# albanie/mcnCrossModalEmotions

Measured on AMD Instinct MI355X. Metric: distillation-step samples/sec (face+audio pair), higher is better.
Workload: dtype f32; 1 GPU; BASELINE config 4 shard: frozen resnet50 teacher fwd + VGGVox student fwd/bwd/SGD; per_gpu_batch=32, global_batch=32, face=224x224x3, teacher_batch=32, spectrogram=512x300x1, parallelism=dp1, weights=random-init (seeded), parameter_server=rccl-capi, streams=teacher one batch ahead on its own stream + wgrad side stream

## Files before the change

### include/xmodal.h

```cpp
#ifndef XMODAL_H
#define XMODAL_H
#include <stddef.h>
#ifdef __cplusplus
extern "C" {
#endif

enum {
  XM_OK = 0,
  XM_EINVAL = 1,
  XM_ENOMEM = 2,
  XM_EHIP = 3,
  XM_ETOOBIG = 4,
  XM_ENOTSUP = 5
};

enum { XM_POOL_MAX = 0, XM_POOL_AVG = 1 };
enum { XM_LOSS_SOFTMAXLOG = 0, XM_LOSS_CLASSERROR = 1 };
enum { XM_AGG_MAX = 0, XM_AGG_MEAN = 1, XM_AGG_PEAK = 2 };
enum { XM_MNR_CONVERGED = 0, XM_MNR_ITERLIMIT = 1, XM_MNR_NOTPD = 2, XM_MNR_BADINPUT = 3 };
enum { XM_ROC_OK = 0, XM_ROC_NAN = 1, XM_ROC_BADINPUT = 2 };

enum { XM_FUSE_RELU = 1, XM_BN_BATCH_MOMENTS = 2, XM_FUSE_SIGMOID = 4 };

int xm_version(void);
const char *xm_last_error(void);
int xm_device_alloc(void **ptr, size_t bytes);
int xm_device_free(void *ptr);
int xm_device_upload(void *dst_device, const void *src_host, size_t bytes);
int xm_device_download(void *dst_host, const void *src_device, size_t bytes);
int xm_device_synchronize(void);
enum { XM_EXEC_SINGLE_STREAM = 1 };
int xm_set_exec_hint(unsigned flags);
unsigned xm_get_exec_hint(void);
int xm_tune_load(const char *path);
int xm_tune_save(const char *path);
int xm_tune_entries(int *total, int *unsaved);
int xm_workspace_reserve(size_t bytes);
size_t xm_workspace_bytes(void);
int xm_workspace_reserve_stream(size_t bytes, void *stream);
unsigned long long xm_workspace_generation(void);
int xm_out_size(int in, int pad_a, int pad_b, int f, int dilate, int stride);

int xm_nnconv_forward(const float *x, int H, int W, int C, int N, const float *f, int FH, int FW,
                      int FC, int K, const float *b, float *y, int sy, int sx, int pt, int pb,
                      int pl, int pr, int dy, int dx, void *stream);
int xm_nnconv_forward_fused(const float *x, int H, int W, int C, int N, const float *f, int FH,
                            int FW, int FC, int K, const float *b, float *y, int sy, int sx,
                            int pt, int pb, int pl, int pr, int dy, int dx, const float *scale,
                            const float *shift, const float *residual, int flags, void *stream);
int xm_nnconv_forward_gated(const float *x, int H, int W, int C, int N, const float *f, int FH, int FW,
                            int FC, int K, const float *b, float *y, int sy, int sx, int pt, int pb,
                            int pl, int pr, int dy, int dx, const float *scale, const float *shift,
                            const float *gate, const float *residual, int flags, void *stream);
int xm_nnconv_forward_moments(const float *x, int H, int W, int C, int N, const float *f, int FH, int FW,
                              int FC, int K, const float *b, float *y, int sy, int sx, int pt, int pb,
                              int pl, int pr, int dy, int dx, float epsilon, float *moments_out, void *stream);
int xm_nnconv_backward(const float *x, int H, int W, int C, int N, const float *f, int FH, int FW,
                       int FC, int K, const float *dzdy, float *dx_out, float *df_out,
                       float *db_out, int sy, int sx, int pt, int pb, int pl, int pr, int dy,
                       int dx, void *stream);
int xm_nnconv_prepare_backward(int H, int W, int C, int N, const float *f, int FH, int FW, int FC, int K,
                               int sy, int sx, int pt, int pb, int pl, int pr, int dy, int dx, void *stream);
int xm_params_changed(void);
int xm_nnconv_backward_accum(const float *x, int H, int W, int C, int N, const float *f, int FH, int FW,
                             int FC, int K, const float *dzdy, float *dx_out, float *df_out,
                             float *db_out, int sy, int sx, int pt, int pb, int pl, int pr, int dy,
                             int dx, const float *dx_accum, void *stream);
int xm_nnconv_backward_filter_bnrelupool(const float *x, int H, int W, int C, int N, int FH, int FW, int FC, int K,
                                         int sy, int sx, int pt, int pb, int pl, int pr, int dy, int dx,
                                         const float *y, const float *bn_g, const float *bn_b, const float *moments,
                                         int train, int ph, int pw, int psy, int psx, int ppt, int ppb, int ppl,
                                         int ppr, const unsigned char *argmax, const float *y_pool,
                                         const float *dzdy_pool, float *dzdf_out, float *dzdb_out, float *dg_out,
                                         float *db_out, void *stream);
int xm_nnconv_bnorm_relu_pool_forward(const float *x, int H, int W, int C, int N, const float *f, int FH, int FW, int FC,
                                      int K, const float *bias, int sy, int sx, int pt, int pb, int pl, int pr, int dy, int dx,
                                      const float *bn_g, const float *bn_b, float epsilon, const float *moments_in, int ph,
                                      int pw, int psy, int psx, int ppt, int ppb, int ppl, int ppr, double *gram,
                                      float *y_pool, unsigned char *argmax, float *moments_out, void *stream);
int xm_stem_gram(const float *x, int H, int W, int N, int FH, int FW, int sy, int sx, int pt, int pb, int pl, int pr,
                 double *gram, void *stream);
int xm_stem_gram_moments(const double *gram, const float *f, const float *b, int FH, int FW, int K, float epsilon,
                         float *moments_out, void *stream);
int xm_nnconv_backward_filter_bnrelupool_gram(const float *x, int H, int W, int C, int N, const float *f, int FH, int FW,
                                              int FC, int K, const float *bias, int sy, int sx, int pt, int pb, int pl,
                                              int pr, int dy, int dx, const float *bn_g, const float *moments, int train,
                                              int ph, int pw, int psy, int psx, int ppt, int ppb, int ppl, int ppr,
                                              const unsigned char *argmax, const float *y_pool, const float *dzdy_pool,
                                              const double *gram, float *df_out, float *dbias_out, float *dg_out,
                                              float *db_out, void *stream);

int xm_nnpool_forward(const float *x, int H, int W, int C, int N, int ph, int pw, int sy, int sx,
                      int pt, int pb, int pl, int pr, int method, float *y, void *stream);
int xm_nnpool_backward(const float *x, int H, int W, int C, int N, int ph, int pw, int sy, int sx,
                       int pt, int pb, int pl, int pr, int method, const float *dzdy, float *dx_out,
                       void *stream);

int xm_nnpool_forward_argmax(const float *x, int H, int W, int C, int N, int ph, int pw, int sy,
                             int sx, int pt, int pb, int pl, int pr, float *y, unsigned char *argmax,
                             void *stream);
int xm_nnpool_backward_argmax(const unsigned char *argmax, int H, int W, int C, int N, int ph, int pw,
                              int sy, int sx, int pt, int pb, int pl, int pr, const float *dzdy,
                              float *dx_out, void *stream);
int xm_nnpool_global_avg_backward_accum(const float *dzdy, const float *accum, float *dx_out, int H, int W, int C, int N,
                                        void *stream);

int xm_nnbnorm_forward(const float *x, int H, int W, int C, int N, const float *g, const float *b,
                       float epsilon, const float *moments_in, float *y, float *moments_out,
                       void *stream);
int xm_nnbnorm_forward_fused(const float *x, int H, int W, int C, int N, const float *g,
                             const float *b, float epsilon, const float *moments_in, float *y,
                             float *moments_out, int flags, void *stream);
int xm_nnbnorm_backward(const float *x, int H, int W, int C, int N, const float *g, const float *b,
                        const float *dzdy, float epsilon, const float *moments_in, float *dx_out,
                        float *dg_out, float *db_out, float *moments_out, void *stream);
int xm_nnbnorm_backward_fused(const float *x, const float *y, int H, int W, int C, int N,
                              const float *g, const float *b, const float *dzdy, float epsilon,
                              const float *moments_in, float *dx_out, float *dg_out, float *db_out,
                              float *moments_out, int flags, void *stream);

int xm_nnbnorm_backward_dxsum(const float *x, const float *y, int H, int W, int C, int N,
                              const float *g, const float *b, const float *dzdy, float epsilon,
                              const float *moments_in, float *dx_out, float *dg_out, float *db_out,
                              float *moments_out, float *dxsum_out, int flags, void *stream);

int xm_nnbnorm_relu_pool_forward(const float *x, int H, int W, int C, int N, const float *g,
                                 const float *b, float epsilon, const float *moments_in, int ph, int pw,
                                 int sy, int sx, int pt, int pb, int pl, int pr, float *y_pool,
                                 unsigned char *argmax, float *moments_out, void *stream);
int xm_nnbnorm_relu_pool_backward(const float *x, int H, int W, int C, int N, const float *g,
                                  const float *b, const float *moments, int train, int ph, int pw,
                                  int sy, int sx, int pt, int pb, int pl, int pr,
                                  const unsigned char *argmax, const float *y_pool, const float *dzdy_pool,
                                  float *dx_out, float *dg_out, float *db_out, float *dxsum_out, void *stream);

int xm_nnrelu(const float *x, size_t n, float leak, const float *dzdy, float *y, void *stream);
int xm_nnsigmoid(const float *x, size_t n, const float *dzdy, float *y, void *stream);
int xm_sum2(const float *a, const float *b, size_t n, int flags, float *y, void *stream);
int xm_scale_axpy(const float *x, int HW, int CN, const float *a, const float *r, int flags,
                  float *y, void *stream);
int xm_scale_backward(const float *x, int HW, int CN, const float *a, const float *dzdy,
                      float *dx_out, float *da_out, void *stream);

int xm_nndropout_forward(const float *x, size_t n, float rate, unsigned long long seed, unsigned long long offset,
                         float *y, float *mask_out, void *stream);
// ... 107 lines not shown
```

### mcncrossmodalemotions_amd/_lib.py

```python
import ctypes as C
import os

import torch

_HERE = os.path.dirname(os.path.abspath(__file__))
SO_PATH = os.environ.get("XM_LIB_PATH") or os.path.join(_HERE, "libxmodal_hip.so")

c_fp = C.c_void_p
_i, _f, _sz, _vp = C.c_int, C.c_float, C.c_size_t, C.c_void_p

SIGNATURES = {
    "xm_version": [],
    "xm_last_error": [],
    "xm_tune_load": [C.c_char_p],
    "xm_tune_save": [C.c_char_p],
    "xm_tune_entries": [C.POINTER(C.c_int), C.POINTER(C.c_int)],
    "xm_set_exec_hint": [C.c_uint],
    "xm_get_exec_hint": [],
    "xm_workspace_reserve": [_sz],
    "xm_workspace_bytes": [],
    "xm_workspace_reserve_stream": [_sz, _vp],
    "xm_workspace_generation": [],
    "xm_device_alloc": [C.POINTER(C.c_void_p), _sz],
    "xm_device_free": [_vp],
    "xm_device_upload": [_vp, _vp, _sz],
    "xm_device_download": [_vp, _vp, _sz],
    "xm_device_synchronize": [],
    "xm_out_size": [_i] * 6,
    "xm_nnconv_forward": [c_fp] + [_i] * 4 + [c_fp] + [_i] * 4 + [c_fp, c_fp] + [_i] * 8 + [_vp],
    "xm_nnconv_forward_moments": [c_fp] + [_i] * 4 + [c_fp] + [_i] * 4 + [c_fp, c_fp] + [_i] * 8 + [_f, c_fp, _vp],
    "xm_nnconv_forward_gated": [c_fp] + [_i] * 4 + [c_fp] + [_i] * 4 + [c_fp, c_fp] + [_i] * 8 +
                               [c_fp, c_fp, c_fp, c_fp, _i, _vp],
    "xm_nnconv_forward_fused": [c_fp] + [_i] * 4 + [c_fp] + [_i] * 4 + [c_fp, c_fp] + [_i] * 8 +
                               [c_fp, c_fp, c_fp, _i, _vp],
    "xm_nnconv_backward": [c_fp] + [_i] * 4 + [c_fp] + [_i] * 4 + [c_fp, c_fp, c_fp, c_fp] +
                          [_i] * 8 + [_vp],
    "xm_nnconv_backward_accum": [c_fp] + [_i] * 4 + [c_fp] + [_i] * 4 + [c_fp, c_fp, c_fp, c_fp] +
                                [_i] * 8 + [c_fp, _vp],
    "xm_nnconv_prepare_backward": [_i] * 4 + [c_fp] + [_i] * 12 + [_vp],
    "xm_nnconv_backward_filter_bnrelupool": [c_fp] + [_i] * 16 + [c_fp, c_fp, c_fp, c_fp] + [_i] * 9 +
                                            [c_fp, c_fp, c_fp, c_fp, c_fp, c_fp, c_fp, _vp],
    "xm_stem_gram": [c_fp] + [_i] * 11 + [_vp, _vp],
    "xm_stem_gram_moments": [_vp, c_fp, c_fp, _i, _i, _i, _f, c_fp, _vp],
    "xm_nnconv_backward_filter_bnrelupool_gram": [c_fp] + [_i] * 4 + [c_fp] + [_i] * 4 + [c_fp] + [_i] * 8 +
                                                 [c_fp, c_fp] + [_i] * 9 + [c_fp, c_fp, c_fp, _vp, c_fp, c_fp, c_fp, c_fp, _vp],
    "xm_nnconv_bnorm_relu_pool_forward": [c_fp] + [_i] * 4 + [c_fp] + [_i] * 4 + [c_fp] + [_i] * 8 + [c_fp, c_fp, _f, c_fp] +
                                         [_i] * 8 + [_vp, c_fp, c_fp, c_fp, _vp],
    "xm_params_changed": [],
    "xm_nnpool_forward": [c_fp] + [_i] * 13 + [c_fp, _vp],
    "xm_nnpool_backward": [c_fp] + [_i] * 13 + [c_fp, c_fp, _vp],
    "xm_nnpool_forward_argmax": [c_fp] + [_i] * 12 + [c_fp, c_fp, _vp],
    "xm_nnpool_backward_argmax": [c_fp] + [_i] * 12 + [c_fp, c_fp, _vp],
    "xm_nnpool_global_avg_backward_accum": [c_fp, c_fp, c_fp, _i, _i, _i, _i, _vp],
    "xm_nnbnorm_forward": [c_fp] + [_i] * 4 + [c_fp, c_fp, _f, c_fp, c_fp, c_fp, _vp],
    "xm_nnbnorm_forward_fused": [c_fp] + [_i] * 4 + [c_fp, c_fp, _f, c_fp, c_fp, c_fp, _i, _vp],
    "xm_nnbnorm_backward": [c_fp] + [_i] * 4 + [c_fp, c_fp, c_fp, _f, c_fp, c_fp, c_fp, c_fp, c_fp,
                                               _vp],
    "xm_nnbnorm_backward_fused": [c_fp, c_fp] + [_i] * 4 + [c_fp, c_fp, c_fp, _f, c_fp, c_fp, c_fp,
                                                             c_fp, c_fp, _i, _vp],
    "xm_nnbnorm_backward_dxsum": [c_fp, c_fp] + [_i] * 4 + [c_fp, c_fp, c_fp, _f, c_fp, c_fp, c_fp,
                                                             c_fp, c_fp, c_fp, _i, _vp],
    "xm_nnbnorm_relu_pool_forward": [c_fp] + [_i] * 4 + [c_fp, c_fp, _f, c_fp] + [_i] * 8 +
                                    [c_fp, c_fp, c_fp, _vp],
    "xm_nnbnorm_relu_pool_backward": [c_fp] + [_i] * 4 + [c_fp, c_fp, c_fp, _i] + [_i] * 8 +
                                     [c_fp, c_fp, c_fp, c_fp, c_fp, c_fp, c_fp, _vp],
    "xm_nndropout_forward": [c_fp, _sz, _f, C.c_ulonglong, C.c_ulonglong, c_fp, c_fp, _vp],
    "xm_nndropout_apply": [c_fp, c_fp, _sz, c_fp, _vp],
    "xm_nnrelu": [c_fp, _sz, _f, c_fp, c_fp, _vp],
    "xm_nnsigmoid": [c_fp, _sz, c_fp, c_fp, _vp],
    "xm_sum2": [c_fp, c_fp, _sz, _i, c_fp, _vp],
    "xm_scale_axpy": [c_fp, _i, _i, c_fp, c_fp, _i, c_fp, _vp],
    "xm_scale_backward": [c_fp, _i, _i, c_fp, c_fp, c_fp, c_fp, _vp],
    "xm_se_squeeze_bn": [c_fp] + [_i] * 4 + [c_fp, c_fp, c_fp, c_fp, _vp],
    "xm_scale_axpy_bn": [c_fp] + [_i] * 4 + [c_fp, c_fp, c_fp, c_fp, c_fp, _i, c_fp, _vp],
    "xm_se_tail_backward_reduce": [c_fp, c_fp, c_fp] + [_i] * 4 + [c_fp, c_fp, c_fp, c_fp, c_fp, _vp],
    "xm_se_tail_backward_apply": [c_fp, c_fp, c_fp] + [_i] * 4 + [c_fp, c_fp, c_fp, c_fp, _i, c_fp, c_fp, c_fp, c_fp, c_fp, _vp],
    "xm_nnsoftmaxt": [c_fp, _i, _i, _i, _f, c_fp, _vp],
    "xm_nnsoftmaxt_backward": [c_fp, c_fp, _i, _i, _i, _f, c_fp, _vp],
    "xm_nnregloss": [c_fp, c_fp, _i, _i, _i, _f, c_fp, c_fp, c_fp, _vp],
    "xm_nnsoftmaxceloss": [c_fp, c_fp, _i, _i, _f, _i, c_fp, c_fp, c_fp, _vp],
    "xm_nnloss": [c_fp, c_fp, _i, _i, _i, c_fp, c_fp, _vp],
    "xm_sgd_update": [c_fp, c_fp, c_fp, _sz, _f, _f, _f, _f, _vp],
    "xm_average_update": [c_fp, c_fp, _sz, _f, _f, _vp],
    "xm_comm_unique_id": [_vp],
    "xm_comm_init": [_vp, _i, _i],
    "xm_allreduce_sum_f32": [c_fp, _sz, _vp],
    "xm_parserv_push": [c_fp, _sz, _vp],
    "xm_parserv_sync": [_vp],
    "xm_comm_count": [C.POINTER(C.c_int)],
    "xm_scale_f32": [c_fp, _sz, _f, _vp],
    "xm_comm_destroy": [],
    "xm_spec_rownorm": [c_fp, _i, _i, _i, c_fp, _vp],
    "xm_spec_magnitude": [c_fp, _i, _i, _i, c_fp, _vp],
    "xm_resample": [c_fp, _i, c_fp, _i, _i, _i, _i, c_fp, _i, _vp],
    "xm_wav_batch": [c_fp, C.c_longlong, c_fp, C.c_longlong, c_fp, c_fp, _i, c_fp, _i, _vp],
    "xm_spec_bucket_batch": [c_fp, C.c_longlong, c_fp, _i, _i, c_fp, _i, _i, _i, c_fp, _vp],
    "xm_aggregate_logits": [c_fp, _i, _i, c_fp, c_fp, _i, _i, c_fp, c_fp, _vp],
    "xm_max_label": [c_fp, _i, _i, c_fp, _vp],
    "xm_class_stats": [c_fp, c_fp, _i, _i, c_fp, c_fp, _vp],
    "xm_normalize_face": [c_fp, _i, _i, _i, C.POINTER(C.c_float), c_fp, _vp],
    "xm_crop_resize_face": [c_fp, _i, _i, _i, _f, _i, _i, C.POINTER(C.c_float), c_fp, _vp],
    "xm_nnaffinegrid": [c_fp, _i, _i, _i, c_fp, _vp],
    "xm_nnaffinegrid_backward": [c_fp, _i, _i, _i, c_fp, _vp],
    "xm_nnbilinearsampler": [c_fp] + [_i] * 4 + [c_fp] + [_i] * 3 + [c_fp, _vp],
    "xm_nnbilinearsampler_backward": [c_fp] + [_i] * 4 + [c_fp] + [_i] * 3 + [c_fp, c_fp, c_fp, _vp],
    "xm_ferplus_batch": [c_fp, _i, _i, _i, c_fp, c_fp, _i, _i, C.POINTER(C.c_float), c_fp, _vp],
    "xm_mnrfit": [c_fp, _i, _i, c_fp, _i, c_fp, c_fp, _i, _i, _i, C.c_double, c_fp, c_fp, c_fp, c_fp, _vp],
    "xm_mnrval": [c_fp, c_fp, _i, _i, _i, c_fp, c_fp, _i, _i, c_fp, c_fp, c_fp, c_fp, _vp],
    "xm_roc": [c_fp, _i, _i, c_fp, c_fp, c_fp, _i, _i, c_fp, c_fp, c_fp, c_fp, c_fp, c_fp, _vp],
    "xm_roc_launches": [],
    "xm_label_hist": [c_fp, _i, _i, _i, c_fp, _vp],
    "xm_group_rows": [c_fp, _i, c_fp, _i, _i, c_fp, c_fp, c_fp, _vp],
    "xm_gather_rows": [c_fp, _i, _i, _i, c_fp, _i, c_fp, _vp],
    "xm_scatter_rows": [c_fp, _i, _i, c_fp, _i, _i, c_fp, _vp],
    "xm_track_peaks": [c_fp, _i, _i, c_fp, c_fp, _i, c_fp, c_fp, c_fp, _vp],
    "xm_jpeg_plan": [_vp, _vp, _i, _vp, _vp, C.c_longlong, _vp, C.c_longlong, _vp],
    "xm_jpeg_decode_batch": [c_fp, C.c_longlong, c_fp, _i, c_fp, _i, c_fp, _i, _i, C.c_longlong, C.c_longlong, C.c_longlong,
                             c_fp, c_fp, _f, _i, _i, C.POINTER(C.c_float), c_fp, _vp],
    "xm_wav_plan": [_vp, _vp, _i, _vp, _i, C.c_longlong, _vp, _vp],
    "xm_wav_decode_batch": [c_fp, C.c_longlong, c_fp, _i, c_fp, C.c_longlong, _vp],
}
_RESTYPES = {"xm_get_exec_hint": C.c_uint, "xm_last_error": C.c_char_p, "xm_workspace_bytes": C.c_size_t,
             "xm_workspace_generation": C.c_ulonglong}
_DEBUG = {"xm_debug_set": [C.c_char_p, _i], "xm_debug_get": [C.c_char_p],
          "xm_prof_enable": [_i],
          "xm_prof_collect": [_i, C.POINTER(C.c_int), C.POINTER(C.c_double), C.POINTER(C.c_double),
                              C.POINTER(C.c_longlong)],
          "xm_prof_collect_bytes": [_i, C.POINTER(C.c_int), C.POINTER(C.c_double)],
          "xm_prof_kernel_name": [_i, C.c_char_p, _i]}
_SWITCHES = {"xm_debug_force_conv_cfg": "conv_cfg", "xm_debug_force_conv_splits": "conv_splits",
# ... 42 lines not shown
```

### mcncrossmodalemotions_amd/csrc/context.cpp

```cpp
#include <cstdlib>
#include <map>
#include <string>
#include <vector>

#include "xm_common.h"

namespace xm {
bool path_on(Path p) {
  static const char *const kEnv[kPathCount] = {"XM_NO_HYBRID",      "XM_NO_HALO",        "XM_NO_SKINNY",     "XM_NO_SKINNY4",
                                               "XM_NO_STEM",        "XM_NO_STEM_WGRAD",  "XM_NO_DMA",        "XM_NO_FUSED_STATS",
                                               "XM_DGRAD_MERGE",    "XM_NO_FAST_TRANSPOSE", "XM_NO_POOL_LDS", "XM_NO_POOL_PATCH",
                                               "XM_NO_POOL_POOLED", "XM_NO_W8", "XM_NO_WGRAD_PATCH", "XM_NO_WGRAD_PATCH_S2", "XM_NO_DGRAD_S2", "XM_NO_STEM3"};
  static bool on[kPathCount];
  static bool read = false;
  if (!read) {
    for (int i = 0; i < kPathCount; ++i) on[i] = getenv(kEnv[i]) == nullptr;
    read = true;
  }
  return on[p];
}

long long env_int(const char *name, long long dflt) {
  const char *e = getenv(name);
  return (e && *e) ? atoll(e) : dflt;
}
double env_double(const char *name, double dflt) {
  const char *e = getenv(name);
  return (e && *e) ? atof(e) : dflt;
}

static char g_err[512] = "";
char *err_buf() { return g_err; }

int fail(int code, const char *fmt, ...) {
  va_list ap;
  va_start(ap, fmt);
  vsnprintf(g_err, sizeof g_err, fmt, ap);
  va_end(ap);
  return code;
}

struct WsBuf {
  void *ptr = nullptr;
  size_t cap = 0;
};
static std::map<hipStream_t, WsBuf> g_ws;
static unsigned long long g_ws_generation = 0;

int ws_get(size_t bytes, void **ptr, hipStream_t stream) {
  WsBuf &w = g_ws[stream];
  if (bytes > w.cap) {
    size_t want = bytes + bytes / 4 + (1u << 20);
    static const bool verbose = getenv("XM_WS_VERBOSE") != nullptr;
    if (verbose) fprintf(stderr, "[xm ws] stream %p grow %zu -> %zu\n", (void *)stream, w.cap, want);
    ++g_ws_generation;
    if (w.ptr) {
      hipError_t e = hipDeviceSynchronize();
      if (e != hipSuccess) return fail(XM_EHIP, "hipDeviceSynchronize -> %s", hipGetErrorString(e));
      (void)hipFree(w.ptr);
      w.ptr = nullptr;
      w.cap = 0;
    }
    hipError_t e = hipMalloc(&w.ptr, want);
    if (e != hipSuccess) {
      w.ptr = nullptr;
      return fail(XM_ENOMEM, "workspace hipMalloc(%zu) -> %s", want, hipGetErrorString(e));
    }
    w.cap = want;
  }
  *ptr = w.ptr;
  return XM_OK;
}

static std::map<std::string, void *> g_tables;

const void *cached_device_table(const void *host, size_t bytes) {
  std::string key((const char *)host, bytes);
  auto it = g_tables.find(key);
  if (it != g_tables.end()) return it->second;
  void *d = nullptr;
  static const bool verbose = getenv("XM_WS_VERBOSE") != nullptr;
  if (verbose) fprintf(stderr, "[xm ws] new device table %zu bytes (#%zu)\n", bytes, g_tables.size());
  if (hipMalloc(&d, bytes) != hipSuccess) return nullptr;
  if (hipMemcpy(d, host, bytes, hipMemcpyHostToDevice) != hipSuccess) {
    (void)hipFree(d);
    return nullptr;
  }
  g_tables.emplace(std::move(key), d);
  return d;
}

}

extern "C" {

int xm_version(void) { return 114; }
const char *xm_last_error(void) { return xm::err_buf(); }

int xm_workspace_reserve(size_t bytes) {
  void *p;
  return xm::ws_get(bytes, &p, nullptr);
}
int xm_workspace_reserve_stream(size_t bytes, void *stream) {
  void *p;
  return xm::ws_get(bytes, &p, (hipStream_t)stream);
}
unsigned long long xm_workspace_generation(void) { return xm::g_ws_generation; }

int xm_device_alloc(void **ptr, size_t bytes) {
  if (!ptr) return xm::fail(XM_EINVAL, "device_alloc: NULL output");
  *ptr = nullptr;
  if (bytes == 0) return XM_OK;
  hipError_t e = hipMalloc(ptr, bytes);
  if (e != hipSuccess) return xm::fail(XM_ENOMEM, "hipMalloc(%zu) -> %s", bytes, hipGetErrorString(e));
  return XM_OK;
}
int xm_device_free(void *ptr) {
  if (!ptr) return XM_OK;
  hipError_t e = hipFree(ptr);
  if (e != hipSuccess) return xm::fail(XM_EHIP, "hipFree -> %s", hipGetErrorString(e));
  return XM_OK;
}
int xm_device_upload(void *dst_device, const void *src_host, size_t bytes) {
  if (bytes == 0) return XM_OK;
  if (!dst_device || !src_host) return xm::fail(XM_EINVAL, "device_upload: NULL pointer");
  hipError_t e = hipMemcpy(dst_device, src_host, bytes, hipMemcpyHostToDevice);
  if (e != hipSuccess) return xm::fail(XM_EHIP, "hipMemcpy(H2D, %zu) -> %s", bytes, hipGetErrorString(e));
  return XM_OK;
}
int xm_device_download(void *dst_host, const void *src_device, size_t bytes) {
  if (bytes == 0) return XM_OK;
  if (!dst_host || !src_device) return xm::fail(XM_EINVAL, "device_download: NULL pointer");
  hipError_t e = hipMemcpy(dst_host, src_device, bytes, hipMemcpyDeviceToHost);
  if (e != hipSuccess) return xm::fail(XM_EHIP, "hipMemcpy(D2H, %zu) -> %s", bytes, hipGetErrorString(e));
  return XM_OK;
}
int xm_device_synchronize(void) {
  hipError_t e = hipDeviceSynchronize();
  if (e != hipSuccess) return xm::fail(XM_EHIP, "hipDeviceSynchronize -> %s", hipGetErrorString(e));
  return XM_OK;
}
size_t xm_workspace_bytes(void) {
  size_t t = 0;
  for (auto &kv : xm::g_ws) t += kv.second.cap;
  return t;
}

int xm_out_size(int in, int pad_a, int pad_b, int f, int dilate, int stride) {
  return xm::out_size(in, pad_a, pad_b, f, dilate, stride);
}
}
```

### mcncrossmodalemotions_amd/csrc/conv.hip

```cpp
#include <dlfcn.h>

#include <algorithm>
#include <climits>
#include <cstdlib>
#include <map>
#include <string>
#include <vector>

#include "conv_kernels.h"
#include "stem_pool_kernels.h"

namespace xm {


__global__ void pad_filter_kernel(const float *__restrict__ f, float *__restrict__ o, int M, int R,
                                  int Rp) {
  size_t i = blockIdx.x * (size_t)blockDim.x + threadIdx.x;
  if (i >= (size_t)M * Rp) return;
  int r = (int)(i % Rp);
  size_t m = i / Rp;
  o[i] = r < R ? f[m * R + r] : 0.f;
}

struct PrepDiv {
  FastDiv tsT, T, tsNT, nT, nU, padc, rows;
};
__global__ void __launch_bounds__(256)
prep_dgrad_filter_kernel(const float *__restrict__ f, float *__restrict__ o, int FH, int FW, int FC,
                         int Kg, int u0, int ustep, int nU, int v0, int vstep, int nV, int lda,
                         int TS, int fold, PrepDiv dv) {
  extern __shared__ float tile[];
  const int T = FH * FW, nT = nU * nV;
  const int c0 = blockIdx.x * TS, k0 = blockIdx.y * TS;
  const int pitch = TS * T + 1;
  for (int i = threadIdx.x; i < TS * TS * T; i += 256) {
    int kl = (int)xm_div((uint32_t)i, dv.tsT), rem = i - kl * (TS * T);
    int cl = (int)xm_div((uint32_t)rem, dv.T);
    int c = c0 + cl, k = k0 + kl;
    tile[kl * pitch + rem] = (c < FC && k < Kg) ? f[(size_t)rem + (size_t)T * (c0 + (size_t)FC * k)] : 0.f;
  }
  __syncthreads();
  for (int i = threadIdx.x; i < TS * TS * nT; i += 256) {
    int cl = (int)xm_div((uint32_t)i, dv.tsNT), rem = i - cl * (TS * nT);
    int kl = (int)xm_div((uint32_t)rem, dv.nT), tt = rem - kl * nT;
    int iv = (int)xm_div((uint32_t)tt, dv.nU), iu = tt - iv * nU;
    int t = (u0 + iu * ustep) + FH * (v0 + iv * vstep);
    int c = c0 + cl, k = k0 + kl;
    if (c < FC && k < Kg) {
      size_t dst = fold ? (size_t)(iu + nU * c) * lda + (size_t)nV * k + iv
                        : (size_t)c * lda + (size_t)nT * k + tt;
      o[dst] = tile[kl * pitch + cl * T + t];
    }
  }
  if (blockIdx.y == 0) {
    const int used = (fold ? nV : nT) * Kg, rows = fold ? nU : 1;
    int padc = lda - used;
    for (int i = threadIdx.x; i < TS * rows * padc; i += 256) {
      int rl = (int)xm_div((uint32_t)i, dv.padc), rr = used + (i - rl * padc);
      int cl = (int)xm_div((uint32_t)rl, dv.rows), ul = rl - cl * rows;
      if (c0 + cl < FC) o[((size_t)(c0 + cl) * rows + ul) * lda + rr] = 0.f;
    }
  }
}

__global__ void __launch_bounds__(256)
transpose_filter_kernel(const float *__restrict__ f, float *__restrict__ o, int K, int R, int ldo) {
  __shared__ float tile[64][65];
  const int r0 = blockIdx.x * 64, k0 = blockIdx.y * 64;
  const int tx = threadIdx.x & 15, ty = threadIdx.x >> 4;
#pragma unroll
  for (int p = 0; p < 4; ++p) {
    const int k = k0 + ty + 16 * p, r = r0 + 4 * tx;
    float4 v = make_float4(0.f, 0.f, 0.f, 0.f);
    if (k < K && r < R) v = *reinterpret_cast<const float4 *>(f + (size_t)k * R + r);
    tile[ty + 16 * p][4 * tx + 0] = v.x;
    tile[ty + 16 * p][4 * tx + 1] = v.y;
    tile[ty + 16 * p][4 * tx + 2] = v.z;
    tile[ty + 16 * p][4 * tx + 3] = v.w;
  }
  __syncthreads();
#pragma unroll
  for (int p = 0; p < 4; ++p) {
    const int r = r0 + ty + 16 * p, k = k0 + 4 * tx;
    if (r < R && k < K) {
      float4 v = make_float4(tile[4 * tx + 0][ty + 16 * p], tile[4 * tx + 1][ty + 16 * p],
                             tile[4 * tx + 2][ty + 16 * p], tile[4 * tx + 3][ty + 16 * p]);
      *reinterpret_cast<float4 *>(o + (size_t)r * ldo + k) = v;
    }
  }
}

template <int ZL>
__global__ void __launch_bounds__(256)
reduce_splits_kernel(const float *__restrict__ part, float *__restrict__ out, size_t total, int splits,
                     size_t splitStride) {
  constexpr int OPB = 256 / ZL;
  const int ol = threadIdx.x % OPB, zl = threadIdx.x / OPB;
  const size_t i = blockIdx.x * (size_t)OPB + ol;
  float s0 = 0.f, s1 = 0.f, s2 = 0.f, s3 = 0.f;
  if (i < total) {
    const float *p = part + i;
    int z = zl;
    for (; z + 3 * ZL < splits; z += 4 * ZL) {
      s0 += p[(size_t)z * splitStride];
      s1 += p[(size_t)(z + ZL) * splitStride];
      s2 += p[(size_t)(z + 2 * ZL) * splitStride];
      s3 += p[(size_t)(z + 3 * ZL) * splitStride];
    }
    for (; z < splits; z += ZL) s0 += p[(size_t)z * splitStride];
  }
  float s = (s0 + s1) + (s2 + s3);
  if (ZL == 1) {
    if (i < total) out[i] = s;
    return;
  }
  __shared__ float red[256];
  red[threadIdx.x] = s;
  __syncthreads();
  if (zl == 0 && i < total) {
    float t = 0.f;
#pragma unroll
    for (int k = 0; k < ZL; ++k) t += red[k * OPB + ol];
    out[i] = t;
  }
}

static void launch_reduce_splits(const float *part, float *out, size_t total, int splits,
                                 size_t splitStride, hipStream_t st) {
  if (splits >= 64)
    hipLaunchKernelGGL(reduce_splits_kernel<16>, dim3((unsigned)((total + 15) / 16)), dim3(256), 0, st,
                       part, out, total, splits, splitStride);
  else if (splits >= 8)
    hipLaunchKernelGGL(reduce_splits_kernel<4>, dim3((unsigned)((total + 63) / 64)), dim3(256), 0, st,
                       part, out, total, splits, splitStride);
  else
    hipLaunchKernelGGL(reduce_splits_kernel<1>, dim3((unsigned)((total + 255) / 256)), dim3(256), 0, st,
                       part, out, total, splits, splitStride);
}

__global__ void __launch_bounds__(256)
bias_grad_partial_kernel(const float *__restrict__ dy, double *__restrict__ part, int HW, int K, int N,
                         int S, FastDiv divRun) {
  int k = blockIdx.x, sp = blockIdx.y;
  double s = 0.0;
  const bool vec = (HW & 3) == 0;
  const int nper = (N - sp + S - 1) / S;
  const int run = vec ? HW >> 2 : HW;
  for (int j = threadIdx.x; j < nper * run; j += 256) {
    const int nn = (int)xm_div((uint32_t)j, divRun), i = j - nn * run;
    const float *p = dy + (size_t)HW * (k + (size_t)K * (sp + nn * S));
    if (vec) {
      float4 v = reinterpret_cast<const float4 *>(p)[i];
      s += ((double)v.x + (double)v.y) + ((double)v.z + (double)v.w);
    } else {
      s += (double)p[i];
    }
  }
  __shared__ double red[4];
  s = xm_wave_sum_d(s);
  if ((threadIdx.x & 63) == 0) red[threadIdx.x >> 6] = s;
  __syncthreads();
  if (threadIdx.x == 0) part[(size_t)k * S + sp] = red[0] + red[1] + red[2] + red[3];
}

__global__ void __launch_bounds__(256)
bias_grad_finalize_kernel(const double *__restrict__ part, float *__restrict__ db, int K, int S) {
  const int k = blockIdx.x * 4 + (threadIdx.x >> 6), lane = threadIdx.x & 63;
  if (k >= K) return;
  double s = 0.0;
  for (int i = lane; i < S; i += 64) s += part[(size_t)k * S + i];
  s = xm_wave_sum_d(s);
  if (lane == 0) db[k] = (float)s;
// ... 957 lines not shown
  bool bigTaps, dma_ok;
};

static ConvGemmArgs forward_args(const Geo &g, int grp, const FwdOperands &o) {
  ConvGemmArgs a{};
  const size_t xoff = (size_t)grp * g.FC * g.H * g.W, yoff = (size_t)grp * g.Kg * g.Ho * g.Wo;
  a.A = o.A + (size_t)grp * g.Kg * o.lda, a.lda = o.lda, a.aBytes = (unsigned)((size_t)g.Kg * o.lda * 4);
  a.X = o.x + xoff, a.xBytes = (unsigned)((x_elements(g) - xoff) * 4), a.xSampleStride = g.H * g.W * g.C;
  a.Y = o.y + yoff, a.taps = o.taps, a.tapStride = (unsigned)((size_t)g.H * g.W * 4);
  a.bias = o.b ? o.b + grp * g.Kg : nullptr;
  a.scale = o.scale ? o.scale + grp * g.Kg : nullptr, a.shift = o.shift ? o.shift + grp * g.Kg : nullptr;
  a.resid = o.resid ? o.resid + yoff : nullptr, a.relu = o.relu;
  a.gate = o.gate ? o.gate + (size_t)grp * g.Kg : nullptr, a.gateStride = g.K;
  a.M = g.Kg, a.Rp = o.Rp, a.Rtrue = g.R;
  a.PI = g.Ho, a.PJ = g.Wo, a.NP = g.Ho * g.Wo * g.N;
  a.divPIJ = make_fastdiv((uint32_t)(g.Ho * g.Wo)), a.divPI = make_fastdiv((uint32_t)g.Ho);
  a.gsy = g.sy, a.gsx = g.sx, a.gh0 = -g.pt, a.gw0 = -g.pl, a.LimH = g.H, a.LimW = g.W;
  a.nU = o.bigTaps ? 1 : g.FH, a.nV = o.bigTaps ? 1 : g.FW;
  a.du0 = 0, a.dus = g.dy, a.dv0 = 0, a.dvs = g.dx;
  a.osy = 1, a.osx = 1, a.oh0 = 0, a.ow0 = 0, a.OH = g.Ho;
  a.oChanStride = g.Ho * g.Wo, a.oSampleStride = g.Ho * g.Wo * g.K, a.divMU = make_fastdiv(1), a.oUStride = 0;
  a.vecStore = ((g.Ho * g.Wo) % 4 == 0 && (((uintptr_t)a.Y | (uintptr_t)a.resid) & 15) == 0) ? 1 : 0;
  a.dmaOk = (o.dma_ok && a.vecStore) ? 1 : 0;
  return a;
}

struct FwdStats {
  bool ok;
  float *part;
  int ncg;
};
static ConvGemmArgs stats_args(const ConvGemmArgs &a, FwdStats &s, int ncg) {
  ConvGemmArgs aa = a;
  s.ncg = ncg;
  if (ncg > 0) aa.statPart = s.part, aa.statNcg = ncg;
  return aa;
}
static int forward_stats_reduce(const FwdStats &s, double *part2, float *moments_out, int K, int NP, float eps, hipStream_t st) {
  const int S = std::max(1, std::min(64, s.ncg / 768));
  hipLaunchKernelGGL(conv_stats_reduce_kernel, dim3((K + 7) / 8, S), dim3(256), 0, st, s.part, moments_out, part2, K, s.ncg, S,
                     (double)NP, eps);
  XM_LAUNCH_CHECK();
  if (S > 1) {
    hipLaunchKernelGGL(conv_stats_finalize2_kernel, dim3((K + 255) / 256), dim3(256), 0, st, part2, moments_out, K, S,
                       (double)NP, eps);
    XM_LAUNCH_CHECK();
  }
  return XM_OK;
}

static int forward_run(const Geo &g, const ConvGemmArgs &a, const float *x, const float *f, int mode, float *slab,
                       FwdStats &s, hipStream_t st) {
  auto gemm = [&](int ci) {
    int sp;
    ci = a.dmaOk ? ci : base_cfg(ci);
    gemm_slab_floats(a, ci, &sp);
    const bool carry = s.ok && sp == 1 && g_force_splits <= 1;
    ConvGemmArgs aa = stats_args(a, s, carry ? (a.NP + kCfgs[ci].bn() - 1) / kCfgs[ci].bn() : 0);
    const int rc_ = launch_gemm(aa, mode, ci, sp, slab, st);
    if (aa.statPart) s.ncg = aa.statNcg;
    return rc_;
  };
  const TuneKey key = tune_key_forward(0, g, a.M, a.NP, a.Rp, mode + (s.ok ? 4 : 0));
  const int ci = tune_cfg(key, pick_cfg(a.M, a.NP, a.Rp / kBK), st, gemm, a.dmaOk ? kNumCfg : kNumBaseCfg, w8_skip(a.M, a.NP));
  if (stem_ok(a, g, x, s.ok)) {
    auto arm = [&](int h) { return h ? launch_stem(stats_args(a, s, s.ok ? stem_grid(a.NP) : 0), f, g.R, st) : gemm(ci); };
    return arm(select_arm(7, key, st, 2, kOneChallenger, kHaloMargin, g_force_stem, arm));
  }
  if (stem3_ok(a, g, x, s.ok)) {
    auto arm = [&](int h) { return h ? launch_stem3(a, f, g.R, st) : gemm(ci); };
    return arm(select_arm(12, key, st, 2, kOneChallenger, kHaloMargin, g_force_stem3, arm));
  }
  ConvGemmArgs ah = a;
  const int hneed = forced_tiling() ? 0 : halo_setup(ah, g.N);
  const bool hok[4] = {true, halo_var_ok(ah, hneed, 0), halo_var_ok(ah, hneed, 1), halo_var_ok(ah, hneed, 2)};
  auto arm = [&](int h) {
    if (!h) return gemm(ci);
    const bool carry = s.ok && halo_splits(ah, h - 1) == 1;
    return launch_halo(stats_args(ah, s, carry ? (a.NP + 127) / 128 : 0), h - 1, slab, st);
  };
  return arm(select_arm(4, key, st, 4, hok, kHaloMargin, halo_forced(hok), arm));
}

static int conv_forward(const float *x, const float *f, const float *b, float *y, const Geo &g,
                        const float *scale, const float *shift, const float *resid, int relu,
                        hipStream_t st, float *moments_out = nullptr, float eps = 0.f, const float *gate = nullptr) {
  const bool padded = (g.pt | g.pb | g.pl | g.pr) != 0;
  const bool bigTaps = g.FH * g.FW > 63;
  if (bigTaps && padded)
    return fail(XM_ENOTSUP, "vl_nnconv: padded filters with more than 63 spatial taps (%dx%d) are not built",
                g.FH, g.FW);
  const int Rp = (g.R + kBK - 1) / kBK * kBK;
  const bool need_pad = (g.R % kBK) != 0 || ((uintptr_t)f & 15);
  const int mode = (padded || Rp != g.R) ? 1 : 0;
  const int NP = g.Ho * g.Wo * g.N;
  const size_t slabf = slab_floats(g.Kg, NP, Rp, kNumCfg, g.FH, g.FW, g.R);
  const bool dma_ok = !need_pad && mode == 0 && g.FH == 1 && g.FW == 1 && g.sy == 1 && g.sx == 1 && g.dy == 1 &&
                      g.dx == 1 && (g.H * g.W) % 4 == 0 && ((uintptr_t)x & 15) == 0 && ((uintptr_t)f & 15) == 0 &&
                      g.R % kBK == 0 && path_on(kPathDma);
  const bool want_stats = moments_out != nullptr && g.G == 1 && path_on(kPathFusedStats);
  const size_t statf = want_stats ? (size_t)2 * g.K * std::max((NP + 31) / 32, stem_grid(NP)) : 0;
  const size_t stat2 = want_stats ? (size_t)2 * g.K * 64 : 0;
  WsCarver ws;
  int rc = ws.init(WsCarver::need(need_pad ? (size_t)g.K * Rp : 0, 4) + WsCarver::need(slabf, 4) +
                       WsCarver::need(statf, 4) + WsCarver::need(stat2, 8), st);
  if (rc) return rc;
  FwdOperands o{x, f, b, scale, shift, resid, gate, y, device_taps(fwd_tap_table(g, Rp, bigTaps)), g.R, Rp, relu, bigTaps, dma_ok};
  if (!o.taps) return fail(XM_ENOMEM, "vl_nnconv: tap table allocation failed");
  if (need_pad) {
    float *Ap = ws.take<float>((size_t)g.K * Rp);
    size_t n = (size_t)g.K * Rp;
    hipLaunchKernelGGL(pad_filter_kernel, dim3((unsigned)((n + 255) / 256)), dim3(256), 0, st, f, Ap,
                       g.K, g.R, Rp);
    XM_LAUNCH_CHECK();
    o.A = Ap;
    o.lda = Rp;
  }
  float *slab = slabf ? ws.take<float>(slabf) : nullptr;
  float *statp = statf ? ws.take<float>(statf) : nullptr;
  double *statp2 = stat2 ? ws.take<double>(stat2) : nullptr;
  bool stats_done = false;
  for (int grp = 0; grp < g.G; ++grp) {
    ConvGemmArgs a = forward_args(g, grp, o);
    FwdStats s{want_stats && a.vecStore && !relu && !resid, statp, 0};
    if (s.ok) a.dmaOk = 0;
    rc = forward_run(g, a, x, f, mode, slab, s, st);
    if (rc) return rc;
    if (s.ncg > 0) {
      rc = forward_stats_reduce(s, statp2, moments_out, g.K, NP, eps, st);
      if (rc) return rc;
      stats_done = true;
    }
  }
  if (moments_out && !stats_done) return bn_batch_moments(y, g.Ho, g.Wo, g.K, g.N, eps, moments_out, st);
  return XM_OK;
}

struct PrepKey {
  const float *f;
  int FH, FW, FC, K, sy, sx, dy, dx, pt, pl, H, W, fold;
  bool operator<(const PrepKey &o) const { return memcmp(this, &o, sizeof(PrepKey)) < 0; }
};
struct PrepEntry {
  float *buf = nullptr;
  size_t bytes = 0;
  unsigned long long version = ~0ull;
  hipEvent_t ev = nullptr;
  hipStream_t st = nullptr;
};
static std::map<PrepKey, PrepEntry> g_prep;
unsigned long long g_param_version = 1;
static PrepKey prep_key(const float *f, const Geo &g, bool fold) {
  PrepKey k;
  memset(&k, 0, sizeof k);
  k.f = f, k.FH = g.FH, k.FW = g.FW, k.FC = g.FC, k.K = g.K, k.sy = g.sy, k.sx = g.sx, k.dy = g.dy, k.dx = g.dx;
  k.pt = g.pt, k.pl = g.pl, k.H = g.H, k.W = g.W, k.fold = fold ? 1 : 0;
  return k;
}

static int g_force_dgrad_s2 = -1;
static bool dgrad_s2_ok(const Geo &g, const float *dzdy, const float *dxo, const float *accum) {
  if (!path_on(kPathDgradS2) || g_force_dgrad_s2 == 0 || forced_tiling()) return false;
  if (!dgrad_s2_can(g, (uintptr_t)dzdy, (uintptr_t)dxo, accum != nullptr)) return false;
  if (g_force_dgrad_s2 == 1) return true;
  static const long long min_blocks = env_int("XM_DGRAD_S2_MIN_BLOCKS", 6 * 768);
  const long long per_sample = (long long)((g.W + 3) / 4 + (g.W + 2) / 4) * (((g.H + 1) / 2 + 63) / 64) * ((g.C + kDgS2Rows - 1) / kDgS2Rows);
  return per_sample * g.N >= min_blocks;
}
static int launch_dgrad_s2(const float *dzdy, const float *f, float *dxo, const Geo &g, hipStream_t st) {
  DgradS2Args a{};
  a.dY = dzdy;
  a.dX = dxo;
  a.dyBytes = (unsigned)((size_t)g.Ho * g.Wo * g.K * g.N * 4);
  a.C = g.C, a.K = g.K, a.H = g.H, a.W = g.W, a.Ho = g.Ho, a.Wo = g.Wo;
  a.pl = g.pl;
  a.nbm = (g.C + kDgS2Rows - 1) / kDgS2Rows;
  a.nkg = g.K / 8;
  a.nmt = ((g.H + 1) / 2 + 63) / 64;
  int blocks = 0;
  for (int px = 0; px < 2; ++px) {
    a.xfirst[px] = ((px - g.pl) % 2 + 2) % 2;
    const int ncols = a.xfirst[px] < g.W ? (g.W - a.xfirst[px] + 1) / 2 : 0;
    a.ncg[px] = (ncols + 1) / 2;
    a.nv[px] = px == 0 ? 3 : 2;
    blocks += a.ncg[px] * a.nmt * a.nbm;
  }
  const size_t fdFloats = (size_t)a.nbm * 2 * 3 * a.nkg * kDgS2Tile;
  WsCarver ws;
  int rc = ws.init(WsCarver::need(fdFloats, 4), st);
  if (rc) return rc;
  float *Fd = ws.take<float>(fdFloats);
  a.Fd = Fd;
  hipLaunchKernelGGL(prep_dgrad_s2_kernel, dim3((unsigned)std::min<size_t>((fdFloats + 255) / 256, 2048)), dim3(256), 0, st, f,
                     Fd, g.C, g.K, a.nbm, a.nkg, g.pl);
  XM_LAUNCH_CHECK();
  {
    ProfScope ps(11 * 100, 2.0 * g.K * (double)g.Ho * g.Wo * g.N * g.R, st,
                 (double)a.dyBytes + 4.0 * g.K * g.R + 4.0 * g.C * (double)g.H * g.W * g.N);
    hipLaunchKernelGGL(conv_dgrad_s2_kernel<1>, dim3((unsigned)(blocks * g.N)), dim3(256), 0, st, a);
  }
  XM_LAUNCH_CHECK();
  return XM_OK;
}

struct DgradFilters {
  char *base = nullptr;
  std::vector<size_t> off;
  float *slab = nullptr;
  float *of(const Geo &g, const DgradClass &c, size_t ic, int grp, bool foldH) const {
    return (float *)(base + off[ic]) + (size_t)grp * g.FC * (foldH ? g.FH : 1) * c.Rp;
  }
};
static bool dgrad_pure_transpose(const Geo &g, const DgradClass &c, bool foldH, const float *f, const float *Ag) {
  const int Rrows = g.FC * (foldH ? g.FH : 1);
  return g.FW == 1 && ((foldH && c.nU == g.FH && c.nV == 1) || (g.FH == 1 && !foldH)) && c.Rp == g.Kg &&
         (Rrows & 3) == 0 && (g.Kg & 3) == 0 && g.G == 1 && (((uintptr_t)f | (uintptr_t)Ag) & 15) == 0 &&
         path_on(kPathFastTranspose);
}
static int launch_dgrad_filter(const float *f, float *Ag, const Geo &g, const DgradClass &c, int grp, bool foldH, hipStream_t st) {
  if (dgrad_pure_transpose(g, c, foldH, f, Ag)) {
    const int Rrows = g.FC * (foldH ? g.FH : 1);
    hipLaunchKernelGGL(transpose_filter_kernel, dim3((Rrows + 63) / 64, (g.Kg + 63) / 64), dim3(256), 0, st, f, Ag,
                       g.Kg, Rrows, c.Rp);
    XM_LAUNCH_CHECK();
    return XM_OK;
  }
  const int T = g.FH * g.FW;
  const int TS = T <= 14 ? 32 : (T <= 56 ? 16 : 8);
  size_t lds = sizeof(float) * (size_t)TS * (TS * T + 1);
  const int nT = c.nU * c.nV, used = (foldH ? c.nV : nT) * g.Kg;
  PrepDiv pd;
  pd.tsT = make_fastdiv((uint32_t)(TS * T)), pd.T = make_fastdiv((uint32_t)T);
  pd.tsNT = make_fastdiv((uint32_t)std::max(1, TS * nT)), pd.nT = make_fastdiv((uint32_t)std::max(1, nT));
  pd.nU = make_fastdiv((uint32_t)std::max(1, c.nU));
  pd.padc = make_fastdiv((uint32_t)std::max(1, c.Rp - used));
  pd.rows = make_fastdiv((uint32_t)(foldH ? std::max(1, c.nU) : 1));
  hipLaunchKernelGGL(prep_dgrad_filter_kernel, dim3((g.FC + TS - 1) / TS, (g.Kg + TS - 1) / TS),
                     dim3(256), lds, st, f + (size_t)g.R * g.Kg * grp, Ag, g.FH, g.FW, g.FC, g.Kg,
                     c.u0, c.ustep, c.nU, c.v0, c.vstep, c.nV, c.Rp, TS, foldH ? 1 : 0, pd);
  XM_LAUNCH_CHECK();
  return XM_OK;
}

static int dgrad_filter_operand(const float *f, const Geo &g, const std::vector<DgradClass> &cls, bool foldH,
                                size_t slab_floats, bool prepare_only, hipStream_t st, WsCarver &ws, DgradFilters &F) {
  size_t abytes = 0;
  for (const DgradClass &c : cls) {
    F.off.push_back(abytes);
    abytes += WsCarver::need((size_t)g.FC * (foldH ? g.FH : 1) * c.Rp * g.G, 4);
  }
  const PrepKey pkey = prep_key(f, g, foldH);
  PrepEntry *pe = nullptr;
  bool have_prepared = false;
  if (prepare_only) {
    pe = &g_prep[pkey];
    if (pe->bytes < abytes) {
      if (pe->buf) {
        XM_HIP(hipDeviceSynchronize());
        (void)hipFree(pe->buf);
      }
      pe->buf = nullptr;
      XM_HIP(hipMalloc((void **)&pe->buf, abytes));
      pe->bytes = abytes;
    }
    if (!pe->ev) XM_HIP(hipEventCreateWithFlags(&pe->ev, hipEventDisableTiming));
  } else {
    auto it = g_prep.find(pkey);
    if (it != g_prep.end() && it->second.version == g_param_version && it->second.bytes >= abytes) {
      pe = &it->second;
      have_prepared = true;
      if (pe->st != st) XM_HIP(hipStreamWaitEvent(st, pe->ev, 0));
    }
  }
  int rc = ws.init((pe ? 0 : abytes) + WsCarver::need(slab_floats, 4), st);
  if (rc) return rc;
  F.base = pe ? (char *)pe->buf : ws.base;
  F.slab = slab_floats ? (float *)(ws.base + (pe ? 0 : abytes)) : nullptr;
  for (size_t ic = 0; ic < cls.size() && !have_prepared; ++ic)
    for (int grp = 0; grp < g.G; ++grp) {
      rc = launch_dgrad_filter(f, F.of(g, cls[ic], ic, grp, foldH), g, cls[ic], grp, foldH, st);
      if (rc) return rc;
    }
  if (prepare_only) {
    pe->version = g_param_version;
    pe->st = st;
    XM_HIP(hipEventRecord(pe->ev, st));
  }
  return XM_OK;
}

struct DgradOperands {
  const float *dzdy, *accum;
  float *dxo;
  bool foldH;
  double pair_total;
};

static ConvGemmArgs dgrad_args(const Geo &g, const DgradClass &c, int grp, const DgradOperands &o, const float *Ag,
                               const int2 *taps) {
  const bool foldH = o.foldH;
  const DgradGather q = dgrad_gather(g, c, foldH);
  ConvGemmArgs a{};
  const size_t xoff = (size_t)grp * g.Kg * g.Ho * g.Wo, yoff = (size_t)grp * g.FC * g.H * g.W;
  a.A = Ag, a.lda = c.Rp, a.taps = taps;
  a.X = o.dzdy + xoff, a.xBytes = (unsigned)((y_elements(g) - xoff) * 4), a.xSampleStride = g.Ho * g.Wo * g.K;
  a.Y = o.dxo + yoff, a.resid = o.accum ? o.accum + yoff : nullptr;
  a.M = foldH ? g.FC * g.FH : g.FC, a.Rp = c.Rp, a.Rtrue = c.Rc;
  a.PI = foldH ? 1 : c.PI, a.PJ = c.PJ, a.NP = a.PI * c.PJ * g.N;
  a.divPIJ = make_fastdiv((uint32_t)(a.PI * c.PJ)), a.divPI = make_fastdiv((uint32_t)a.PI);
  a.gsy = 1, a.gsx = 1, a.gh0 = q.gh0, a.gw0 = q.gw0, a.LimH = g.Ho, a.LimW = g.Wo;
  a.nU = q.nU, a.nV = c.nV, a.du0 = q.du0, a.dus = q.dus, a.dv0 = q.dv0, a.dvs = q.dvs;
  a.osy = foldH ? 0 : g.sy, a.oh0 = foldH ? 0 : c.hi0;
  a.osx = g.sx, a.ow0 = c.wi0, a.OH = g.H;
  a.oChanStride = g.H * g.W, a.oSampleStride = g.H * g.W * g.C;
  a.divMU = make_fastdiv(foldH ? (uint32_t)g.FH : 1u), a.oUStride = foldH ? 1 : 0;
  a.vecStore = (!foldH && g.sy == 1 && g.sx == 1 && (c.PI * c.PJ) % 4 == 0 && c.PI == g.H &&
                c.PJ == g.W && (((uintptr_t)a.Y | (uintptr_t)a.resid) & 15) == 0) ? 1 : 0;
  a.algoFlops = 2.0 * g.Ho * g.Wo * (double)g.N * g.Kg * g.R * ((double)a.NP * c.Rc) / o.pair_total;
  return a;
}

static bool dgrad_as_skinny_fc(const Geo &g, bool pure_t, bool foldH, const float *accum, Geo &gs) {
  if (!pure_t || foldH || accum || g.FH != 1 || g.sy != 1 || g.sx != 1 || (g.pt | g.pb | g.pl | g.pr) != 0 ||
      g.H * g.W != 1 || (g.FC & 3) != 0 || g.N > 512 || forced_tiling())
    return false;
  gs = g;
  gs.C = gs.FC = g.Kg;
  gs.K = gs.Kg = g.FC;
  gs.R = g.Kg;
  return fc_skinny_ok(gs, true);
}

static int dgrad_run_class(const Geo &g, const DgradClass &c, const ConvGemmArgs &a, bool foldH, float *slab, hipStream_t st) {
  auto gemm = [&](int ci) {
    int sp;
    gemm_slab_floats(a, ci, &sp);
    ConvGemmArgs aa = a;
    return launch_gemm(aa, 1, ci, sp, slab, st);
  };
  const TuneKey key = tune_key_class_dgrad(1, g, c, a.M, a.NP, a.PI);
  const int ci = tune_cfg(key, pick_cfg(a.M, a.NP, c.Rp / kBK), st, gemm, kNumBaseCfg, w8_skip(a.M, a.NP));
  ConvGemmArgs ah = a;
  const int hneed = (!forced_tiling() && !foldH) ? halo_setup_padded(ah, g.N) : 0;
  const bool hok[4] = {true, halo_var_ok(ah, hneed, 0), halo_var_ok(ah, hneed, 1), halo_var_ok(ah, hneed, 2)};
  auto arm = [&](int h) { return h ? launch_halo(ah, h - 1, slab, st) : gemm(ci); };
  return arm(select_arm(5, key, st, 4, hok, kHaloMargin, halo_forced(hok), arm));
}

static bool dgrad_merge_ok(const Geo &g, const std::vector<DgradClass> &cls, bool foldH) {
  if (g.G != 1 || foldH || cls.size() < 2 || cls.size() > 4 || g_force_splits != 0 || !path_on(kPathDgradMerge)) return false;
  long long tiles = 0;
  for (const DgradClass &c : cls) tiles += (long long)((g.FC + 127) / 128) * (((long long)c.PI * c.PJ * g.N + 255) / 256);
  return tiles >= 512;
}

static int dgrad_run_merged(const Geo &g, const std::vector<ConvGemmArgs> &merged, hipStream_t st) {
  auto gemm = [&](int ci) { return launch_gemm_multi(merged, ci, st); };
  long long npSum = 0;
  int rpMax = 0;
  for (const ConvGemmArgs &a : merged) {
    npSum += a.NP;
    rpMax = std::max(rpMax, a.Rp);
  }
  const TuneKey key = tune_key_merged_dgrad(3, g, merged[0].M, npSum, rpMax, (int)merged.size());
  const int ci = tune_cfg(key, pick_cfg(merged[0].M, npSum, rpMax / kBK), st, gemm, kNumBaseCfg, w8_skip(merged[0].M, npSum));
  std::vector<ConvGemmArgs> mh = merged;
  bool hok[4] = {true, g_force_cfg < 0, g_force_cfg < 0, g_force_cfg < 0};
  for (ConvGemmArgs &a : mh) {
    const int need = hok[1] || hok[2] || hok[3] ? halo_setup_padded(a, g.N) : 0;
    for (int v = 0; v < 3; ++v) hok[v + 1] = hok[v + 1] && halo_var_ok(a, need, v);
  }
  if (!hok[3]) {
    bool all = g_force_cfg < 0;
    for (ConvGemmArgs &a : mh) {
      ConvGemmArgs t = a;
      const int need = all ? halo_setup_padded(t, g.N) : 0;
      all = all && need > 0 && need <= 1024 && t.M % 96 == 0;
    }
    hok[3] = all && !hok[2];
  }
  auto arm = [&](int h) { return h ? launch_halo_multi(mh, h - 1, st) : gemm(ci); };
  return arm(select_arm(6, key, st, 4, hok, kHaloMargin, halo_forced(hok), arm));
}

static int conv_dgrad(const float *f, const float *dzdy, float *dxo, const Geo &g, hipStream_t st,
                      const float *accum = nullptr, bool prepare_only = false) {
  if (dgrad_s2_ok(g, dzdy, dxo, accum)) {
    if (prepare_only) return XM_OK;
    return launch_dgrad_s2(dzdy, f, dxo, g, st);
  }
  const bool foldH = dgrad_fold_h(g);
  bool covers_all = true;
  const std::vector<DgradClass> cls = dgrad_classes(g, foldH, &covers_all);
  if (!prepare_only && (!covers_all || cls.empty())) {
    const size_t bytes = sizeof(float) * x_elements(g);
    if (accum)
      XM_HIP(hipMemcpyAsync(dxo, accum, bytes, hipMemcpyDeviceToDevice, st));
    else
      XM_HIP(hipMemsetAsync(dxo, 0, bytes, st));
  }
  if (cls.empty()) return XM_OK;
  for (const DgradClass &c : cls)
    if (c.nU * c.nV > 63)
      return fail(XM_ENOTSUP, "vl_nnconv: more than 63 spatial taps per stride class is not built");
  size_t slab_max = 0;
  for (const DgradClass &c : cls)
    slab_max = std::max(slab_max, slab_floats(foldH ? g.FC * g.FH : g.FC, (foldH ? 1 : c.PI) * c.PJ * g.N, c.Rp, kNumBaseCfg,
                                              foldH ? 0 : c.nU, foldH ? 0 : c.nV, c.Rc));
  WsCarver ws;
  DgradFilters F;
  int rc = dgrad_filter_operand(f, g, cls, foldH, slab_max, prepare_only, st, ws, F);
  if (rc) return rc;
  std::vector<const int2 *> taps;
  for (const DgradClass &c : cls) {
    taps.push_back(device_taps(dgrad_tap_table(g, c, foldH)));
    if (!taps.back()) return fail(XM_ENOMEM, "vl_nnconv: tap table allocation failed");
  }
  if (prepare_only) return XM_OK;
  DgradOperands o{dzdy, accum, dxo, foldH, 0.0};
  for (const DgradClass &c : cls) o.pair_total += (double)(foldH ? 1 : c.PI) * c.PJ * g.N * c.Rc;
  const bool merge = dgrad_merge_ok(g, cls, foldH);
  std::vector<ConvGemmArgs> merged;
  for (size_t ic = 0; ic < cls.size(); ++ic)
    for (int grp = 0; grp < g.G; ++grp) {
      const DgradClass &c = cls[ic];
      const float *Ag = F.of(g, c, ic, grp, foldH);
      Geo gs;
      if (dgrad_as_skinny_fc(g, dgrad_pure_transpose(g, c, foldH, f, Ag), foldH, accum, gs)) {
        rc = fc_skinny_forward(dzdy, Ag, nullptr, dxo, gs, 0, st);
        if (rc) return rc;
        continue;
      }
      const ConvGemmArgs a = dgrad_args(g, c, grp, o, Ag, taps[ic]);
      if (merge) {
        merged.push_back(a);
        continue;
      }
      rc = dgrad_run_class(g, c, a, foldH, F.slab, st);
      if (rc) return rc;
    }
  return merge ? dgrad_run_merged(g, merged, st) : XM_OK;
}

static int wgrad_run(const float *x, const float *dzdy, float *dfo, const Geo &g, int ci, float *part,
                     hipStream_t st) {
  ci = wgrad_cfg(ci);
  const Cfg &c = kCfgs[ci];
  const int NP = g.Ho * g.Wo * g.N;
  const int nkt = (NP + kBK - 1) / kBK;
  const int nbm = (g.Kg + c.bm() - 1) / c.bm(), nbn = (g.R + c.bn() - 1) / c.bn();
  const int Rn = nbn * c.bn();
  const int tiles = nbm * nbn;
  const int slots = 256 * (c.bm() * c.bn() >= 128 * 128 ? 2 : (c.bm() * c.bn() >= 64 * 128 ? 3 : 6));
  int splits = std::max(1, std::min(nkt / 8, slots / tiles));
  splits = std::min(splits, 1024);
  int tps = (nkt + splits - 1) / splits;
  splits = (nkt + tps - 1) / tps;
  const int4 *taps = device_taps(wgrad_tap_table(g, Rn));
  if (!taps) return fail(XM_ENOMEM, "vl_nnconv: tap table allocation failed");
  const size_t slab = (size_t)g.Kg * g.R;
  for (int grp = 0; grp < g.G; ++grp) {
    WgradArgs a{};
    const size_t xoff = (size_t)grp * g.FC * g.H * g.W, doff = (size_t)grp * g.Kg * g.Ho * g.Wo;
    float *dst = dfo + (size_t)grp * g.Kg * g.R;
    a.dY = dzdy + doff, a.dyBytes = (unsigned)((y_elements(g) - doff) * 4);
    a.X = x + xoff, a.xBytes = (unsigned)((x_elements(g) - xoff) * 4);
    a.out = splits > 1 ? part : dst, a.taps = taps;
    a.M = g.Kg, a.R = g.R, a.Rn = Rn, a.ldo = g.R;
    a.Ho = g.Ho, a.Wo = g.Wo, a.NP = NP;
    a.divHW = make_fastdiv((uint32_t)(g.Ho * g.Wo)), a.divHo = make_fastdiv((uint32_t)g.Ho);
    a.sy = g.sy, a.sx = g.sx, a.pt = g.pt, a.pl_ = g.pl, a.H = g.H, a.W = g.W;
    a.xSampleStride = g.H * g.W * g.C, a.dyChanStride = g.Ho * g.Wo, a.dySampleStride = g.Ho * g.Wo * g.K;
    a.nbm = nbm, a.nbn = nbn, a.tilesPerSplit = tps, a.nkt = nkt, a.splitStride = slab;
    {
// ... 180 lines not shown
    return arm(select_arm(9, key, st, 2, kOneChallenger, 0.01f, g_force_wgrad_patch, arm));
  }
  if (wgrad_patch_s2_ok(g, x, dzdy)) {
    auto arm = [&](int h) { return h ? launch_wgrad_patch_s2(x, dzdy, dfo, g, part, max_splits, st) : run(ci); };
    return arm(select_arm(10, key, st, 2, kOneChallenger, 0.01f, g_force_wgrad_patch_s2, arm));
  }
  return run(ci);
}

static bool stem_pool_ok(const Geo &g, const float *x) { return path_on(kPathStem) && stem_pool_can(g, (uintptr_t)x); }

static int stem_pool_units(const Geo &g) { return g.N * ((g.Wo + 1) / 2) * ((g.Ho + 255) / 256); }
static void stem_pool_args(StemPoolArgs &a, const float *x, const Geo &g) {
  a.X = x, a.M = g.Kg, a.R = g.R, a.nU = g.FH, a.nV = g.FW, a.PI = g.Ho, a.PJ = g.Wo;
  const int G = (g.Ho + 255) / 256;
  a.divJG = make_fastdiv((uint32_t)(((g.Wo + 1) / 2) * G)), a.divG = make_fastdiv((uint32_t)G);
  a.gsx = g.sx, a.gh0 = -g.pt, a.gw0 = -g.pl, a.LimH = g.H, a.LimW = g.W, a.xSampleStride = g.H * g.W;
}

static int stem_pool_grid(int nunits, int occ) { return std::min(256 * occ, (nunits + 7) / 8 * 8); }
static size_t stem_gram_need(const Geo &g) {
  return WsCarver::need((size_t)stem_pool_grid(stem_pool_units(g), 3) * 64 * 64, 4);
}

static int launch_stem_gram(WsCarver &ws, const float *x, const Geo &g, double *gram, hipStream_t st) {
  StemPoolArgs a{};
  stem_pool_args(a, x, g);
  const int nunits = stem_pool_units(g), grid = stem_pool_grid(nunits, 3);
  a.part = ws.take<float>((size_t)grid * 64 * 64);
  static bool attr_done = false;
  if (!attr_done) {
    XM_HIP(hipFuncSetAttribute((const void *)stem_gram_kernel<2>, hipFuncAttributeMaxDynamicSharedMemorySize, kSpGramSmem));
    XM_HIP(hipFuncSetAttribute((const void *)stem_gram_kernel<1>, hipFuncAttributeMaxDynamicSharedMemorySize, kSpGramSmem));
    attr_done = true;
  }
  {
    ProfScope ps(13 * 100, 2.0 * (g.R + 1) * (g.R + 1) * (double)g.Ho * g.Wo * g.N, st, 4.0 * g.H * g.W * g.N);
    if (g.sy == 2) hipLaunchKernelGGL(stem_gram_kernel<2>, dim3(grid), dim3(256), kSpGramSmem, st, a, nunits);
    else hipLaunchKernelGGL(stem_gram_kernel<1>, dim3(grid), dim3(256), kSpGramSmem, st, a, nunits);
  }
  XM_LAUNCH_CHECK();
  hipLaunchKernelGGL(stem_gram_reduce_kernel, dim3(64), dim3(1024), 0, st, a.part, gram, grid);
  XM_LAUNCH_CHECK();
  return XM_OK;
}

}

using namespace xm;

static int norm_tri(int v) { return v < 0 ? -1 : (v ? 1 : 0); }
static const struct DebugSwitch {
  const char *name;
  int *value;
  int (*normalise)(int);
} kDebugSwitches[] = {
    {"conv_cfg", &g_force_cfg, [](int v) { return (v >= 0 && v < kNumCfg) ? v : -1; }},
    {"conv_splits", &g_force_splits, [](int v) { return v > 0 ? v : 0; }},
    {"conv_halo", &g_force_halo, [](int v) { return v < 0 ? -1 : std::min(v, 3); }},
    {"conv_stem", &g_force_stem, norm_tri},         {"conv_stem3", &g_force_stem3, norm_tri},
    {"wgrad_patch", &g_force_wgrad_patch, norm_tri}, {"wgrad_patch_s2", &g_force_wgrad_patch_s2, norm_tri},
    {"dgrad_s2", &g_force_dgrad_s2, norm_tri},
    {"spec_blocks", &g_spec_blocks, [](int v) { return v > 0 ? v : 0; }},
};
static const DebugSwitch *debug_switch(const char *key) {
  for (const DebugSwitch &s : kDebugSwitches)
    if (key && strcmp(key, s.name) == 0) return &s;
  return nullptr;
}

extern "C" {

int xm_debug_set(const char *key, int value) {
  if (const DebugSwitch *s = debug_switch(key)) {
    const int old = *s->value;
    *s->value = s->normalise(value);
    return old;
  }
  if (key && strcmp(key, "comm_single") == 0) return comm_force_single(value);
  return INT_MIN;
}
int xm_debug_get(const char *key) {
  if (key && strcmp(key, "num_conv_cfgs") == 0) return kNumCfg;
  const DebugSwitch *s = debug_switch(key);
  return s ? *s->value : INT_MIN;
}

int xm_set_exec_hint(unsigned flags) {
  if (flags & ~(unsigned)XM_EXEC_SINGLE_STREAM) return fail(XM_EINVAL, "xm_set_exec_hint: unknown flag bits 0x%x", flags);
  g_exec_hint = flags;
  return XM_OK;
}
unsigned xm_get_exec_hint(void) { return g_exec_hint; }


int xm_tune_load(const char *path) {
  g_tune_loaded = true;
  return tune_load_file(path && path[0] ? path : tune_default_path().c_str());
}
int xm_tune_save(const char *path) {
  tune_load_once();
  std::string p = path && path[0] ? std::string(path) : tune_default_path();
  std::string tmp = p + ".tmp";
  FILE *fp = fopen(tmp.c_str(), "w");
  if (!fp) return fail(XM_EINVAL, "xm_tune_save: cannot write %s", tmp.c_str());
  fprintf(fp, "xmodal-tune 1 rev=%d cfgs=%d\n", XM_TUNE_REV, kNumCfg);
  for (auto &kv : g_tuned) {
    const TuneKey &k = kv.first;
    fprintf(fp, "%d %d %d %d %d %d %d %d %d %d\n", k.kind, k.M, k.NP, k.Rp, k.mode, k.a, k.b, k.c, k.d, kv.second);
  }
  fclose(fp);
  if (rename(tmp.c_str(), p.c_str()) != 0) return fail(XM_EINVAL, "xm_tune_save: rename to %s failed", p.c_str());
  g_tune_new = 0;
  return XM_OK;
}
int xm_tune_entries(int *total, int *unsaved) {
  tune_load_once();
  if (total) *total = (int)g_tuned.size();
  if (unsaved) *unsaved = g_tune_new;
  return XM_OK;
}
#ifdef XM_DEBUG_CYCLES
int xm_debug_conv_cycles(int on, unsigned long long *out, int nblocks) {
  const size_t bytes = 4096 * 4 * sizeof(unsigned long long);
  if (on && !g_dbg_cycles) {
    if (hipMalloc((void **)&g_dbg_cycles, bytes) != hipSuccess) return XM_ENOMEM;
    (void)hipMemset(g_dbg_cycles, 0, bytes);
  }
  if (out && g_dbg_cycles)
    (void)hipMemcpy(out, g_dbg_cycles, (size_t)std::min(nblocks, 4096) * 32, hipMemcpyDeviceToHost);
  if (!on && g_dbg_cycles) {
    (void)hipFree(g_dbg_cycles);
    g_dbg_cycles = nullptr;
  }
  return XM_OK;
}
#endif

int xm_prof_enable(int on) {
  if (on) {
    for (auto &r : g_prof) {
      g_event_pool.push_back(r.start);
      g_event_pool.push_back(r.stop);
    }
    g_prof.clear();
  }
  g_prof_on = on != 0;
  return XM_OK;
}

static size_t prof_slot(std::vector<int> &ks, int key) {
  const size_t i = std::find(ks.begin(), ks.end(), key) - ks.begin();
  if (i == ks.size()) ks.push_back(key);
  return i;
}

int xm_prof_collect(int cap, int *keys, double *total_ms, double *total_flops, long long *launches) {
  std::vector<int> ks;
  std::vector<double> ms, fl;
  std::vector<long long> cnt;
  for (auto &r : g_prof) {
    float t = 0.f;
    if (hipEventElapsedTime(&t, r.start, r.stop) != hipSuccess) continue;
    const size_t i = prof_slot(ks, r.key);
    if (i == ms.size()) ms.push_back(0), fl.push_back(0), cnt.push_back(0);
    ms[i] += t;
// ... 73 lines not shown
  }
  int ci = (kind == 0 || kind == 2) ? (key % 100) / 2 : (key % 100) / 4;
  if (ci < 0 || ci >= kNumCfg) return XM_EINVAL;
  const Cfg &c = kCfgs[ci];
  if (kind == 0 && is_dma_cfg(ci))
    snprintf(buf, len, "conv_gemm_dma_kernel<%d, %d, %d, %d, %d>", c.tm, c.tn, c.wgm, c.wgn,
             ci == kNumBaseCfg ? XM_DMA_NST7 : ci == kNumBaseCfg + 1 ? 3 : ci == kNumBaseCfg + 2 ? XM_DMA_NST9 : XM_DMA_NST10);
  else if (kind == 0)
    snprintf(buf, len, "conv_gemm_kernel<%d, %d, %d, %d, %d>", c.tm, c.tn, c.wgm, c.wgn, key % 2);
  else if (kind == 2)
    snprintf(buf, len, "conv_gemm_multi_kernel<%d, %d, %d, %d>", c.tm, c.tn, c.wgm, c.wgn);
  else
    snprintf(buf, len, "conv_wgrad_kernel<%d, %d, %d, %d, %d>", c.tm, c.tn, c.wgm, c.wgn, 1 << (key % 4));
  return XM_OK;
}

int xm_nnconv_forward_fused(const float *x, int H, int W, int C, int N, const float *f, int FH,
                            int FW, int FC, int K, const float *b, float *y, int sy, int sx,
                            int pt, int pb, int pl, int pr, int dy, int dx, const float *scale,
                            const float *shift, const float *residual, int flags, void *stream) {
  Geo g;
  int rc = make_geo(g, H, W, C, N, FH, FW, FC, K, sy, sx, pt, pb, pl, pr, dy, dx);
  if (rc) return rc;
  if (!x || !f || !y) return fail(XM_EINVAL, "vl_nnconv: NULL tensor");
  if ((scale == nullptr) != (shift == nullptr))
    return fail(XM_EINVAL, "vl_nnconv(fused): scale and shift must be given together");
  if ((flags & XM_FUSE_RELU) && (flags & XM_FUSE_SIGMOID))
    return fail(XM_EINVAL, "vl_nnconv(fused): relu and sigmoid are exclusive");
  hipStream_t st = (hipStream_t)stream;
  if (!residual && fc_skinny_ok(g))
    return fc_skinny_forward(x, f, b, y, g, (flags & XM_FUSE_SIGMOID) ? 2 : ((flags & XM_FUSE_RELU) ? 1 : 0), st, scale,
                             shift);
  rc = conv_forward(x, f, b, y, g, scale, shift, residual, (flags & XM_FUSE_RELU) ? 1 : 0, st);
  if (rc || !(flags & XM_FUSE_SIGMOID)) return rc;
  return xm_nnsigmoid(y, (size_t)g.Ho * g.Wo * g.K * g.N, nullptr, y, stream);
}

int xm_nnconv_forward_moments(const float *x, int H, int W, int C, int N, const float *f, int FH, int FW,
                              int FC, int K, const float *b, float *y, int sy, int sx, int pt, int pb,
                              int pl, int pr, int dy, int dx, float epsilon, float *moments_out, void *stream) {
  Geo g;
  int rc = make_geo(g, H, W, C, N, FH, FW, FC, K, sy, sx, pt, pb, pl, pr, dy, dx);
  if (rc) return rc;
  if (!x || !f || !y || !moments_out) return fail(XM_EINVAL, "vl_nnconv(+moments): NULL tensor");
  hipStream_t st = (hipStream_t)stream;
  if (fc_skinny_ok(g)) {
    rc = fc_skinny_forward(x, f, b, y, g, 0, st);
    return rc ? rc : bn_batch_moments(y, g.Ho, g.Wo, g.K, g.N, epsilon, moments_out, st);
  }
  return conv_forward(x, f, b, y, g, nullptr, nullptr, nullptr, 0, st, moments_out, epsilon);
}

int xm_nnconv_forward_gated(const float *x, int H, int W, int C, int N, const float *f, int FH, int FW,
                            int FC, int K, const float *b, float *y, int sy, int sx, int pt, int pb,
                            int pl, int pr, int dy, int dx, const float *scale, const float *shift,
                            const float *gate, const float *residual, int flags, void *stream) {
  Geo g;
  int rc = make_geo(g, H, W, C, N, FH, FW, FC, K, sy, sx, pt, pb, pl, pr, dy, dx);
  if (rc) return rc;
  if (!x || !f || !y || !gate) return fail(XM_EINVAL, "vl_nnconv(gated): NULL tensor");
  if ((scale == nullptr) != (shift == nullptr))
    return fail(XM_EINVAL, "vl_nnconv(gated): scale and shift must be given together");
  if (flags & XM_FUSE_SIGMOID) return fail(XM_ENOTSUP, "vl_nnconv(gated): sigmoid epilogue is not built");
  return conv_forward(x, f, b, y, g, scale, shift, residual, (flags & XM_FUSE_RELU) ? 1 : 0, (hipStream_t)stream,
                      nullptr, 0.f, gate);
}

int xm_nnconv_forward(const float *x, int H, int W, int C, int N, const float *f, int FH, int FW,
                      int FC, int K, const float *b, float *y, int sy, int sx, int pt, int pb,
                      int pl, int pr, int dy, int dx, void *stream) {
  return xm_nnconv_forward_fused(x, H, W, C, N, f, FH, FW, FC, K, b, y, sy, sx, pt, pb, pl, pr, dy,
                                 dx, nullptr, nullptr, nullptr, 0, stream);
}

int xm_nnconv_prepare_backward(int H, int W, int C, int N, const float *f, int FH, int FW, int FC, int K,
                               int sy, int sx, int pt, int pb, int pl, int pr, int dy, int dx, void *stream) {
  Geo g;
  int rc = make_geo(g, H, W, C, N, FH, FW, FC, K, sy, sx, pt, pb, pl, pr, dy, dx);
  if (rc) return rc;
  if (!f) return fail(XM_EINVAL, "vl_nnconv: F is NULL");
  return conv_dgrad(f, nullptr, nullptr, g, (hipStream_t)stream, nullptr, true);
}

int xm_params_changed(void) {
  ++g_param_version;
  return XM_OK;
}

int xm_nnconv_backward_filter_bnrelupool(const float *x, int H, int W, int C, int N, int FH, int FW, int FC, int K, int sy,
                                         int sx, int pt, int pb, int pl, int pr, int dy, int dx, const float *y,
                                         const float *bn_g, const float *bn_b, const float *moments, int train, int ph,
                                         int pw, int psy, int psx, int ppt, int ppb, int ppl, int ppr,
                                         const unsigned char *argmax, const float *y_pool, const float *dzdy_pool,
                                         float *df_out, float *dbias_out, float *dg_out, float *db_out, void *stream) {
  Geo g;
  int rc = make_geo(g, H, W, C, N, FH, FW, FC, K, sy, sx, pt, pb, pl, pr, dy, dx);
  if (rc) return rc;
  if (!x || !y || !bn_g || !bn_b || !moments || !argmax || !dzdy_pool || !df_out)
    return fail(XM_EINVAL, "vl_nnconv(filter derivative through bnorm+relu+pool): NULL tensor");
  hipStream_t st = (hipStream_t)stream;
  const int pHo = out_size(g.Ho, ppt, ppb, ph, 1, psy), pWo = out_size(g.Wo, ppl, ppr, pw, 1, psx);
  const bool ok = g_force_stem != 0 && stem_wgrad_can(g, (uintptr_t)x, (uintptr_t)y) && g.K == g.Kg && y_pool != nullptr &&
                  pool3x3s2_unpadded(ph, pw, psy, psx, ppt, ppb, ppl, ppr) && (g.Ho & 1) == 0 && pHo >= 1 && pWo >= 1 &&
                  (!dbias_out || g.R < 64) && fits_i32_bytes((size_t)pHo * pWo * g.K * g.N);
  if (!ok)
    return fail(XM_ENOTSUP, "vl_nnconv(filter derivative through bnorm+relu+pool): geometry not covered by the fused kernel");
  const int grid = stem_grid(g.Ho * g.Wo * g.N);
  WsCarver ws;
  rc = ws.init(WsCarver::need((size_t)6 * g.K, 4) + WsCarver::need((size_t)grid * 96 * 64, 4) + bnpool_sums_need(g.K, g.N), st);
  if (rc) return rc;
  float *rowc = ws.take<float>((size_t)6 * g.K);
  float *spart = ws.take<float>((size_t)grid * 96 * 64);
  rc = bnpool_backward_sums(ws, y, g.Ho, g.Wo, g.K, g.N, bn_g, bn_b, moments, train, ph, pw, psy, psx, ppt, ppb, ppl, ppr,
                            argmax, y_pool, dzdy_pool, dg_out, db_out, rowc, st);
  if (rc) return rc;
  StemBnp bnp{dzdy_pool, argmax, rowc, pHo, pWo, dbias_out};
  return launch_stem_wgrad(x, y, df_out, g, spart, grid, st, &bnp);
}

int xm_stem_gram(const float *x, int H, int W, int N, int FH, int FW, int sy, int sx, int pt, int pb, int pl, int pr,
                 double *gram, void *stream) {
  Geo g;
  int rc = make_geo(g, H, W, 1, N, FH, FW, 1, 1, sy, sx, pt, pb, pl, pr, 1, 1);
  if (rc) return rc;
  if (!x || !gram) return fail(XM_EINVAL, "xm_stem_gram: NULL tensor");
  if (!stem_pool_ok(g, x)) return fail(XM_ENOTSUP, "xm_stem_gram: geometry not covered");
  hipStream_t st = (hipStream_t)stream;
  WsCarver ws;
  rc = ws.init(stem_gram_need(g), st);
  if (rc) return rc;
  return launch_stem_gram(ws, x, g, gram, st);
}

int xm_stem_gram_moments(const double *gram, const float *f, const float *b, int FH, int FW, int K, float epsilon,
                         float *moments_out, void *stream) {
  if (!gram || !f || !moments_out) return fail(XM_EINVAL, "xm_stem_gram_moments: NULL tensor");
  if (FH * FW < 1 || FH * FW > 63 || K < 1) return fail(XM_EINVAL, "xm_stem_gram_moments: bad shape");
  hipLaunchKernelGGL(stem_gram_moments_kernel, dim3(K), dim3(64), 0, (hipStream_t)stream, gram, f, b, K, FH * FW,
                     (double)epsilon, moments_out);
  XM_LAUNCH_CHECK();
  return XM_OK;
}

int xm_nnconv_bnorm_relu_pool_forward(const float *x, int H, int W, int C, int N, const float *f, int FH, int FW, int FC,
                                      int K, const float *bias, int sy, int sx, int pt, int pb, int pl, int pr, int dy, int dx,
                                      const float *bn_g, const float *bn_b, float epsilon, const float *moments_in, int ph,
                                      int pw, int psy, int psx, int ppt, int ppb, int ppl, int ppr, double *gram,
                                      float *y_pool, unsigned char *argmax, float *moments_out, void *stream) {
  Geo g;
  int rc = make_geo(g, H, W, C, N, FH, FW, FC, K, sy, sx, pt, pb, pl, pr, dy, dx);
  if (rc) return rc;
  if (!x || !f || !bn_g || !bn_b || !y_pool || !argmax || (!moments_in && (!gram || !moments_out)))
    return fail(XM_EINVAL, "vl_nnconv + bnorm + relu + pool (fused forward): NULL tensor");
  hipStream_t st = (hipStream_t)stream;
  const int pHo = out_size(g.Ho, ppt, ppb, ph, 1, psy), pWo = out_size(g.Wo, ppl, ppr, pw, 1, psx);
  const long long pooled = (long long)pHo * pWo * g.K * g.N;
  const bool ok = path_on(kPathStem) && g_force_stem != 0 &&
                  fused_stem_can(kFusedStemForward, g, (uintptr_t)x, ph, pw, psy, psx, ppt, ppb, ppl, ppr, pHo, pWo, (uintptr_t)y_pool);
  if (!ok)
    return fail(XM_ENOTSUP, "vl_nnconv + bnorm + relu + pool (fused forward): geometry not covered by the fused kernel");
  const float *moments = moments_in;
  if (!moments_in) {
    WsCarver ws;
    rc = ws.init(stem_gram_need(g), st);
    if (rc) return rc;
    rc = launch_stem_gram(ws, x, g, gram, st);
    if (rc) return rc;
    hipLaunchKernelGGL(stem_gram_moments_kernel, dim3(g.K), dim3(64), 0, st, gram, f, bias, g.K, g.R, (double)epsilon,
// ... 157 lines not shown
```

### mcncrossmodalemotions_amd/csrc/misc.hip

```cpp
#include "xm_common.h"

namespace xm {
extern unsigned long long g_param_version;
}

namespace xm {

static unsigned ew_grid(size_t work_items) {
  size_t b = (work_items + 255) / 256;
  if (b > 256 * 8) b = 256 * 8;
  if (b < 1) b = 1;
  return (unsigned)b;
}

enum { OP_RELU_F, OP_RELU_B, OP_SIG_F, OP_SIG_B, OP_SUM, OP_SUM_RELU };

template <int OP>
__device__ __forceinline__ float ew_op(float a, float b, float leak) {
  if (OP == OP_RELU_F) return a > 0.f ? a : leak * a;
  if (OP == OP_RELU_B) return a > 0.f ? b : leak * b;
  if (OP == OP_SIG_F) return 1.f / (1.f + expf(-a));
  if (OP == OP_SIG_B) {
    float s = 1.f / (1.f + expf(-a));
    return b * s * (1.f - s);
  }
  if (OP == OP_SUM) return a + b;
  return fmaxf(a + b, 0.f);
}

template <int OP, bool BINARY>
__global__ void __launch_bounds__(256)
ew_kernel(const float *__restrict__ a, const float *__restrict__ b, float *__restrict__ y, size_t n,
          float leak, int vec) {
  size_t stride = (size_t)gridDim.x * 256;
  size_t i0 = blockIdx.x * (size_t)256 + threadIdx.x;
  if (vec) {
    size_t n4 = n >> 2;
    for (size_t i = i0; i < n4; i += stride) {
      float4 av = reinterpret_cast<const float4 *>(a)[i];
      float4 bv = BINARY ? reinterpret_cast<const float4 *>(b)[i] : make_float4(0, 0, 0, 0);
      float4 o;
      o.x = ew_op<OP>(av.x, bv.x, leak);
      o.y = ew_op<OP>(av.y, bv.y, leak);
      o.z = ew_op<OP>(av.z, bv.z, leak);
      o.w = ew_op<OP>(av.w, bv.w, leak);
      reinterpret_cast<float4 *>(y)[i] = o;
    }
    for (size_t i = (n4 << 2) + i0; i < n; i += stride)
      y[i] = ew_op<OP>(a[i], BINARY ? b[i] : 0.f, leak);
  } else {
    for (size_t i = i0; i < n; i += stride) y[i] = ew_op<OP>(a[i], BINARY ? b[i] : 0.f, leak);
  }
}

template <int OP, bool BINARY>
static int ew_launch(const float *a, const float *b, float *y, size_t n, float leak, hipStream_t st) {
  if (n == 0) return XM_OK;
  if (!a || !y || (BINARY && !b)) return fail(XM_EINVAL, "elementwise op: NULL tensor");
  int vec = ((((uintptr_t)a | (uintptr_t)b | (uintptr_t)y) & 15) == 0) ? 1 : 0;
  hipLaunchKernelGGL((ew_kernel<OP, BINARY>), dim3(ew_grid(vec ? n / 4 + 1 : n)), dim3(256), 0, st, a,
                     b, y, n, leak, vec);
  XM_LAUNCH_CHECK();
  return XM_OK;
}

__global__ void __launch_bounds__(256)
scale_axpy_kernel(const float *__restrict__ x, const float *__restrict__ a,
                  const float *__restrict__ r, float *__restrict__ y, FastDiv divHW, size_t total,
                  int relu) {
  size_t stride = (size_t)gridDim.x * 256;
  for (size_t i = blockIdx.x * (size_t)256 + threadIdx.x; i < total; i += stride) {
    uint32_t plane = xm_div((uint32_t)i, divHW);
    float v = a[plane] * x[i] + (r ? r[i] : 0.f);
    if (relu) v = fmaxf(v, 0.f);
    y[i] = v;
  }
}

__global__ void __launch_bounds__(256)
se_squeeze_bn_kernel(const float *__restrict__ u, const float *__restrict__ g, const float *__restrict__ b,
                     const float *__restrict__ mom, int HW, int C, int planes, float *__restrict__ gp) {
  const int plane = blockIdx.x * 4 + (threadIdx.x >> 6);
  if (plane >= planes) return;
  const int lane = threadIdx.x & 63, c = plane % C;
  const float *p = u + (size_t)plane * HW;
  const float sc = g[c] / mom[C + c], mu = mom[c], bb = b[c];
// ... 621 lines not shown
  else
    hipLaunchKernelGGL(se_tail_apply_kernel<false>, dim3(grid), dim3(256), 0, st, y, dzdy, u, gate, dgp, g, moments, sums,
                       make_fastdiv((uint32_t)HW), C, total, m, train, dz_out, du_out);
  XM_LAUNCH_CHECK();
  return XM_OK;
}

int xm_scale_backward(const float *x, int HW, int CN, const float *a, const float *dzdy,
                      float *dx_out, float *da_out, void *stream) {
  if (HW <= 0 || CN <= 0) return fail(XM_EINVAL, "scale: empty tensor");
  if (!x || !a || !dzdy) return fail(XM_EINVAL, "scale: NULL tensor");
  hipLaunchKernelGGL(scale_bwd_kernel, dim3((CN + 3) / 4), dim3(256), 0, (hipStream_t)stream, x, a,
                     dzdy, dx_out, da_out, HW, CN);
  XM_LAUNCH_CHECK();
  return XM_OK;
}

int xm_nnsoftmaxt(const float *x, int HW, int C, int N, float temperature, float *y, void *stream) {
  if (HW <= 0 || C <= 0 || N <= 0) return fail(XM_EINVAL, "vl_nnsoftmaxt: empty tensor");
  if (!(temperature > 0.f)) return fail(XM_EINVAL, "vl_nnsoftmaxt: temperature must be > 0");
  int cols = HW * N;
  hipLaunchKernelGGL(softmaxt_kernel, dim3((cols + 127) / 128), dim3(128), 0, (hipStream_t)stream, x, y,
                     HW, C, N, temperature);
  XM_LAUNCH_CHECK();
  return XM_OK;
}

int xm_nnsoftmaxt_backward(const float *x, const float *dzdy, int HW, int C, int N, float temperature,
                           float *dx, void *stream) {
  if (HW <= 0 || C <= 0 || N <= 0) return fail(XM_EINVAL, "vl_nnsoftmaxt: empty tensor");
  if (!x || !dzdy || !dx) return fail(XM_EINVAL, "vl_nnsoftmaxt: NULL tensor");
  if (!(temperature > 0.f)) return fail(XM_EINVAL, "vl_nnsoftmaxt: temperature must be > 0");
  int cols = HW * N;
  hipLaunchKernelGGL(softmaxt_bwd_kernel, dim3((cols + 127) / 128), dim3(128), 0, (hipStream_t)stream, x,
                     dzdy, dx, HW, C, N, temperature);
  XM_LAUNCH_CHECK();
  return XM_OK;
}

int xm_nnsoftmaxceloss(const float *x, const float *p, int C, int N, float temperature,
                       int logit_targets, const float *instance_weights, const float *dzdy,
                       float *y, void *stream) {
  if (C <= 0 || N <= 0) return fail(XM_EINVAL, "vl_nnsoftmaxceloss: empty tensor");
  if (C > 64) return fail(XM_ENOTSUP, "vl_nnsoftmaxceloss: more than 64 classes (%d)", C);
  if (!(temperature > 0.f)) return fail(XM_EINVAL, "vl_nnsoftmaxceloss: temperature must be > 0");
  if (!x || !p || !y) return fail(XM_EINVAL, "vl_nnsoftmaxceloss: NULL tensor");
  hipLaunchKernelGGL(softmaxceloss_kernel, dim3(1), dim3(256), 0, (hipStream_t)stream, x, p, C, N,
                     temperature, logit_targets, instance_weights, dzdy, y);
  XM_LAUNCH_CHECK();
  return XM_OK;
}

int xm_nnregloss(const float *x, const float *t, int E, int N, int kind, float sigma,
                 const float *instance_weights, const float *dzdy, float *y, void *stream) {
  if (E <= 0 || N <= 0) return fail(XM_EINVAL, "regression loss: empty tensor");
  if (too_big(E, N)) return fail(XM_ETOOBIG, "regression loss: tensor too large");
  if (kind != XM_REGLOSS_EUCLIDEAN && kind != XM_REGLOSS_HUBER)
    return fail(XM_ENOTSUP, "regression loss: kind %d not built (euclidean, huber)", kind);
  if (kind == XM_REGLOSS_HUBER && !(sigma > 0.f)) return fail(XM_EINVAL, "vl_nnhuberloss: sigma must be > 0");
  if (!x || !t || !y) return fail(XM_EINVAL, "regression loss: NULL tensor");
  size_t n = (size_t)E * N;
  size_t nb = (n + 255) / 256;
  unsigned grid = dzdy ? (unsigned)(nb < 4096 ? nb : 4096) : 1u;
  hipLaunchKernelGGL(regloss_kernel, dim3(grid), dim3(256), 0, (hipStream_t)stream, x, t, E, N, kind,
                     sigma, instance_weights, dzdy, y);
  XM_LAUNCH_CHECK();
  return XM_OK;
}

int xm_nnloss(const float *x, const float *labels, int C, int N, int loss, const float *dzdy,
              float *y, void *stream) {
  if (C <= 0 || N <= 0) return fail(XM_EINVAL, "vl_nnloss: empty tensor");
  if (loss != XM_LOSS_SOFTMAXLOG && loss != XM_LOSS_CLASSERROR)
    return fail(XM_ENOTSUP, "vl_nnloss: loss type %d not built (softmaxlog, classerror only)", loss);
  if (!x || !labels || !y) return fail(XM_EINVAL, "vl_nnloss: NULL tensor");
  hipLaunchKernelGGL(nnloss_kernel, dim3(1), dim3(256), 0, (hipStream_t)stream, x, labels, C, N, loss,
                     dzdy, y);
  XM_LAUNCH_CHECK();
  return XM_OK;
}

int xm_sgd_update(float *w, float *m, const float *der, size_t n, float lr, float momentum,
                  float weight_decay, float batch, void *stream) {
  ++xm::g_param_version;
  if (n == 0) return XM_OK;
  if (!w || !m || !der) return fail(XM_EINVAL, "sgd: NULL tensor");
  if (!(batch > 0.f)) return fail(XM_EINVAL, "sgd: batch must be > 0");
  int vec = ((((uintptr_t)w | (uintptr_t)m | (uintptr_t)der) & 15) == 0) ? 1 : 0;
  hipLaunchKernelGGL(sgd_kernel, dim3(ew_grid(vec ? n / 4 + 1 : n)), dim3(256), 0, (hipStream_t)stream,
                     w, m, der, n, lr, momentum, weight_decay, 1.0f / batch, vec);
  XM_LAUNCH_CHECK();
  return XM_OK;
}

int xm_scale_f32(float *x, size_t n, float a, void *stream) {
  if (n == 0) return XM_OK;
  if (!x) return fail(XM_EINVAL, "scale: NULL tensor");
  hipLaunchKernelGGL(scale_kernel, dim3((unsigned)((n + 255) / 256)), dim3(256), 0, (hipStream_t)stream, x, n, a);
  XM_LAUNCH_CHECK();
  return XM_OK;
}

int xm_nndropout_forward(const float *x, size_t n, float rate, unsigned long long seed, unsigned long long offset,
                         float *y, float *mask_out, void *stream) {
  if (n == 0) return XM_OK;
  if (!x || !y) return fail(XM_EINVAL, "vl_nndropout: NULL tensor");
  if (!(rate >= 0.f && rate < 1.f)) return fail(XM_EINVAL, "vl_nndropout: rate must be in [0, 1)");
  const size_t groups = (n + 3) / 4;
  hipLaunchKernelGGL(dropout_fwd_kernel, dim3((unsigned)((groups + 255) / 256)), dim3(256), 0, (hipStream_t)stream, x, n,
                     rate, 1.f / (1.f - rate), seed, offset, y, mask_out);
  XM_LAUNCH_CHECK();
  return XM_OK;
}

int xm_nndropout_apply(const float *x, const float *mask, size_t n, float *y, void *stream) {
  if (n == 0) return XM_OK;
  if (!x || !mask || !y) return fail(XM_EINVAL, "vl_nndropout: NULL tensor");
  hipLaunchKernelGGL(mul_kernel, dim3((unsigned)((n + 255) / 256)), dim3(256), 0, (hipStream_t)stream, x, mask, n, y);
  XM_LAUNCH_CHECK();
  return XM_OK;
}

int xm_average_update(float *w, const float *der, size_t n, float lr, float nworkers, void *stream) {
  ++xm::g_param_version;
  if (n == 0) return XM_OK;
  if (!w || !der) return fail(XM_EINVAL, "average update: NULL tensor");
  hipLaunchKernelGGL(average_kernel, dim3((unsigned)((n + 255) / 256)), dim3(256), 0,
                     (hipStream_t)stream, w, der, n, lr, 1.0f / nworkers);
  XM_LAUNCH_CHECK();
  return XM_OK;
}

__global__ void __launch_bounds__(256)
spec_magnitude_kernel(const float *__restrict__ reim, float *__restrict__ out, int Wo, int B, int N) {
  __shared__ float tile[32][33];
  const int n = blockIdx.z, j0 = blockIdx.x * 32, b0 = blockIdx.y * 32;
  const int tx = threadIdx.x & 31, ty = threadIdx.x >> 5;
  const float *src = reim + (size_t)Wo * 2 * B * n;
  for (int r = ty; r < 32; r += 8) {
    int b = b0 + r, j = j0 + tx;
    float v = 0.f;
    if (b < B && j < Wo) {
      float re = src[j + (size_t)Wo * b], im = src[j + (size_t)Wo * (B + b)];
      v = sqrtf(re * re + im * im);
    }
    tile[r][tx] = v;
  }
  __syncthreads();
  float *dst = out + (size_t)B * Wo * n;
  for (int r = ty; r < 32; r += 8) {
    int j = j0 + r, b = b0 + tx;
    if (b < B && j < Wo) dst[b + (size_t)B * j] = tile[tx][r];
  }
}

int xm_spec_magnitude(const float *reim, int Wo, int B, int N, float *out, void *stream) {
  if (Wo <= 0 || B <= 0 || N <= 0) return fail(XM_EINVAL, "spec_magnitude: empty input");
  if (N > 65535) return fail(XM_ETOOBIG, "spec_magnitude: more than 65535 clips per call");
  if (too_big(Wo, 2 * B, N)) return fail(XM_ETOOBIG, "spec_magnitude: tensor too large");
  if (!reim || !out) return fail(XM_EINVAL, "spec_magnitude: NULL tensor");
  hipLaunchKernelGGL(spec_magnitude_kernel, dim3((Wo + 31) / 32, (B + 31) / 32, N), dim3(256), 0,
                     (hipStream_t)stream, reim, out, Wo, B, N);
  XM_LAUNCH_CHECK();
  return XM_OK;
}

__global__ void __launch_bounds__(256)
resample_kernel(const float *__restrict__ x, int Lx, const float *__restrict__ h, int Lh, int p, int q, int delay,
                float *__restrict__ y, int Ly) {
  const int j = blockIdx.x * 256 + threadIdx.x;
  if (j >= Ly) return;
  const long long t0 = (long long)(j + delay) * q;
  long long klo = (t0 - (Lh - 1) + p - 1) / p;
  if (t0 - (Lh - 1) < 0) klo = 0;
  long long khi = t0 / p;
  if (khi > Lx - 1) khi = Lx - 1;
  float acc = 0.f;
  for (long long k = klo; k <= khi; ++k) acc = fmaf(h[t0 - k * p], x[k], acc);
  y[j] = acc;
}

int xm_resample(const float *x, int Lx, const float *h, int Lh, int p, int q, int delay, float *y, int Ly, void *stream) {
  if (Lx <= 0 || Lh <= 0 || p <= 0 || q <= 0 || delay < 0 || Ly < 0) return fail(XM_EINVAL, "resample: bad sizes");
  if (Ly == 0) return XM_OK;
  if (!x || !h || !y) return fail(XM_EINVAL, "resample: NULL tensor");
  hipLaunchKernelGGL(resample_kernel, dim3((Ly + 255) / 256), dim3(256), 0, (hipStream_t)stream, x, Lx, h, Lh, p, q, delay,
                     y, Ly);
  XM_LAUNCH_CHECK();
  return XM_OK;
}

struct WavClip {
  int p, q;
  float gain;
  float pad;
};
constexpr int kWavMaxRatio = 1 << 20;
constexpr float kWavBeta2Over4 = 6.25f;

__device__ __forceinline__ float wav_i0(float y) {
  const float c[15] = {1.000000000e+00f, 1.000000000e+00f, 2.500000000e-01f, 2.777777778e-02f, 1.736111111e-03f,
                       6.944444444e-05f, 1.929012346e-06f, 3.936759889e-08f, 6.151187327e-10f, 7.594058428e-12f,
                       7.594058428e-14f, 6.276081346e-16f, 4.358389823e-18f, 2.578928890e-20f, 1.315780046e-22f};
  float s = c[14];
#pragma unroll
  for (int k = 13; k >= 0; --k) s = fmaf(s, y, c[k]);
  return s;
}

__device__ __forceinline__ float wav_tap(int m, int r, int odd, int P, float invP, float P_over_pi, int half, float kb) {
  const int rr = 2 * r > P ? P - r : r;
  float s = sinpif((float)rr * invP);
  s = odd ? -s : s;
// ... 305 lines not shown
```

### mcncrossmodalemotions_amd/dagnn.py

```python
import os
from collections import OrderedDict

import numpy as np
import torch

from . import vl


class Param:
    def __init__(self, name, value=None, learningRate=1.0, weightDecay=1.0, trainMethod="gradient"):
        self.name = name
        self.value = value
        self.der = None
        self.learningRate = learningRate
        self.weightDecay = weightDecay
        self.trainMethod = trainMethod
        self.fanout = 0


class Var:
    def __init__(self, name):
        self.name = name
        self.value = None
        self.der = None
# ... 337 lines not shown

    def reset(self):
        super().reset()
        if self._correct is not None:
            self._correct.zero_()
            self._population.zero_()

    def forward(self, inputs, params):
        y = vl.vl_nnloss(inputs[0], inputs[1], loss="classerror")
        if self._correct is None:
            self._correct = vl.mat_zeros(self.numClasses, 1, device=inputs[0].device)
            self._population = vl.mat_zeros(self.numClasses, 1, device=inputs[0].device)
        vl.class_stats(inputs[0], inputs[1], self._correct, self._population)
        self.lastValue = y
        self.lastN = int(inputs[0].shape[3]) if inputs[0].dim() > 3 else 1
        self.numAveraged += self.lastN
        return [y]

    @property
    def classDist(self):
        if self._population is None:
            return np.zeros(self.numClasses)
        return vl.to_numpy(self._population).ravel().astype(np.float64)

    @property
    def average(self):
        if self._correct is None:
            return np.zeros(self.numClasses)
        c = vl.to_numpy(self._correct).ravel().astype(np.float64)
        return c / np.maximum(self.classDist, 1.0)

    def backward(self, inputs, params, derOutputs):
        return [None, None], []


class _LayerRec:
    def __init__(self, name, block, inputs, outputs, params):
        self.name = name
        self.block = block
        self.inputs = list(inputs)
        self.outputs = list(outputs)
        self.params = list(params)


class DagNN:

    def __init__(self):
        self.layers = []
        self.vars = OrderedDict()
        self.params = OrderedDict()
        self.meta = {}
        self.mode = "normal"
        self.conserveMemory = True
        self.accumulateParamDers = False
        self.fuse = True
        self.fuseStats = os.environ.get("XM_NO_FUSED_STATS") is None
        self.wgradAfterDgrad = os.environ.get("XM_WGRAD_AFTER_DGRAD") is not None
        self.fuseBiasDer = os.environ.get("XM_NO_FUSED_BIASDER") is None
        self.fuseStemBackward = os.environ.get("XM_NO_FUSED_STEM_BWD") is None
        self.fuseStemGram = os.environ.get("XM_NO_STEM_GRAM") is None
        self.fuseStemForward = os.environ.get("XM_NO_STEM_FWD") is None
        self.fuseForkSums = os.environ.get("XM_NO_FORK_SUMS") is None
        self.fuseSE = os.environ.get("XM_NO_FUSED_SE") is None
        self.foldSEReduce = os.environ.get("XM_NO_SE_FOLD_FC") is None
        self.fuseSETrain = os.environ.get("XM_NO_FUSED_SE_BWD") is None
        self.wgradStream = None
        self.gradHook = None
        self.markHook = None
        self.bwdHooks = {}
        self._side_pending = False
        self._training = False
        self.prepareBackward = os.environ.get("XM_NO_PREPARE") is None
        self.device = None
        self._flat = None
        self._gen = [0]

    @property
    def paramGeneration(self):
        return self._gen[0]

    @paramGeneration.setter
    def paramGeneration(self, v):
        self._gen[0] = int(v)

    def addLayer(self, name, block, inputs, outputs, params=()):
        if isinstance(inputs, str):
            inputs = [inputs]
        if isinstance(outputs, str):
            outputs = [outputs]
        if isinstance(params, str):
            params = [params]
        if any(l.name == name for l in self.layers):
            raise ValueError("There is already a layer with name '%s'." % name)
        block.net = self
        self.layers.append(_LayerRec(name, block, inputs, outputs, params))
        for p in params:
            if p not in self.params:
                self.params[p] = Param(p)
        self.rebuild()
        return self

    def insertLayerAfter(self, prev, name, block, inputs, outputs, params=()):
        self.addLayer(name, block, inputs, outputs, params)
        rec = self.layers.pop()
        self.layers.insert(self.getLayerIndex(prev) + 1, rec)
        self.rebuild()
        return self

    def setLayerInputs(self, name, inputs):
        self.layers[self.getLayerIndex(name)].inputs = [inputs] if isinstance(inputs, str) else list(inputs)
        self.rebuild()
        return self

    def removeLayer(self, name):
        names = [name] if isinstance(name, str) else list(name)
        self.layers = [l for l in self.layers if l.name not in names]
        self.rebuild()

    def renameVar(self, old, new):
        for l in self.layers:
            l.inputs = [new if v == old else v for v in l.inputs]
            l.outputs = [new if v == old else v for v in l.outputs]
        self.rebuild()

    def rebuild(self):
        old = self.vars
        self.vars = OrderedDict()
        for p in self.params.values():
            p.fanout = 0
        for i, l in enumerate(self.layers):
            l.block.layerIndex = i
            l.block.net = self
            for v in l.inputs:
                self.vars.setdefault(v, old.get(v) or Var(v))
            for v in l.outputs:
                self.vars.setdefault(v, old.get(v) or Var(v))
        for v in self.vars.values():
            v.fanin = v.fanout = 0
        for l in self.layers:
            for v in l.inputs:
                self.vars[v].fanout += 1
            for v in l.outputs:
                self.vars[v].fanin += 1
            for p in l.params:
                self.params[p].fanout += 1
        used = {p for l in self.layers for p in l.params}
        for p in list(self.params):
            if p not in used:
                del self.params[p]

    def replica(self):
        import copy
        r = DagNN()
        r.meta, r.mode, r.fuse, r.device = self.meta, self.mode, self.fuse, self.device
        r.conserveMemory = self.conserveMemory
        for l in self.layers:
            r.layers.append(_LayerRec(l.name, copy.copy(l.block), l.inputs, l.outputs, l.params))
        r.params = self.params
        r._gen = self._gen
        r.rebuild()
        for name, v in self.vars.items():
            r.vars[name].precious = v.precious
        return r

    def getLayerIndex(self, name):
        for i, l in enumerate(self.layers):
            if l.name == name:
                return i
        return None

    def getLayer(self, name):
        i = self.getLayerIndex(name)
        return None if i is None else self.layers[i]

    def getVarIndex(self, name):
        return list(self.vars).index(name) if name in self.vars else None

    def getParamIndex(self, name):
        return list(self.params).index(name) if name in self.params else None

    def getInputs(self):
        return [v.name for v in self.vars.values() if v.fanin == 0]

    def getOutputs(self):
        return [v.name for v in self.vars.values() if v.fanout == 0]

    def initParams(self, seed=0):
        rng = np.random.default_rng(seed)
        for l in self.layers:
            vals = l.block.initParams(rng)
            for pname, v in zip(l.params, vals):
                self.params[pname].value = v
                if isinstance(l.block, BatchNorm):
                    k = l.params.index(pname)
                    p = self.params[pname]
                    p.weightDecay = 0.0
                    p.learningRate = (2.0, 1.0, 0.1)[k]
                    p.trainMethod = "average" if k == 2 else "gradient"
                elif isinstance(l.block, Conv) and l.params.index(pname) == 1:
                    self.params[pname].weightDecay = 0.0
                    self.params[pname].learningRate = 2.0
        self._flat = None
        self.paramGeneration += 1

    def move(self, device="gpu"):
        if device != "gpu":
            raise RuntimeError("this build has no CPU path (dag.move('cpu'))")
        self.device = torch.device("cuda", torch.cuda.current_device())
        for p in self.params.values():
            if p.value is not None and not isinstance(p.value, torch.Tensor):
                p.value = vl.from_numpy(p.value, self.device)
        return self

    def pack_params(self):
        self.move("gpu")
        groups = OrderedDict()
        for p in self.params.values():
            key = (p.trainMethod, float(p.learningRate), float(p.weightDecay))
            groups.setdefault(key, []).append(p)
        total = sum(int(p.value.numel() + 3) // 4 * 4 for ps in groups.values() for p in ps)
        val = torch.zeros(total, dtype=torch.float32, device=self.device)
        der = torch.zeros(total, dtype=torch.float32, device=self.device)
        mom = torch.zeros(total, dtype=torch.float32, device=self.device)
        off = 0
        segs = []
        for key, ps in groups.items():
            start = off
            for p in ps:
                n = int(p.value.numel())
                shp = tuple(int(s) for s in p.value.shape)
                view = val[off:off + n].view(tuple(reversed(shp))).permute(*reversed(range(len(shp))))
                view.copy_(p.value)
                p.value = view
                p.der = der[off:off + n].view(tuple(reversed(shp))).permute(*reversed(range(len(shp))))
                p._flat_off = off
                off += (n + 3) // 4 * 4
            segs.append((key, start, off))
        self._flat = FlatParams(val, der, mom, segs)
        self.paramGeneration += 1
        return self._flat

    def eval(self, inputs, derOutputs=None, input_events=None):
        if not isinstance(inputs, dict):
            inputs = {inputs[i]: inputs[i + 1] for i in range(0, len(inputs), 2)}
        if derOutputs is not None and not isinstance(derOutputs, dict):
            derOutputs = {derOutputs[i]: derOutputs[i + 1] for i in range(0, len(derOutputs), 2)}
        for v in self.vars.values():
            if not v.precious:
                v.value = None
            v.der = None
        for k, t in inputs.items():
            if k not in self.vars:
                continue
            self.vars[k].value = t
        plan = self._plan(derOutputs is not None)
        self._training = derOutputs is not None
        if self._training and self.wgradStream is not None:
            self.wgradStream.wait_stream(torch.cuda.current_stream())
        pending = dict(input_events or {})
        mark = self.markHook or (lambda label: None)
        mark("fwd0")
        for step in plan:
            if pending:
                recs = [step.rec] + [getattr(step, n) for n in ("relu_rec", "pool_rec", "bn_rec", "sum_rec")
                                     if getattr(step, n, None) is not None]
                for rec in recs:
                    for v in rec.inputs:
                        ev = pending.pop(v, None)
                        if ev is not None:
                            torch.cuda.current_stream().wait_event(ev)
            step.forward(self)
        mark("fwd1")
        if derOutputs is None:
            return
        for k, d in derOutputs.items():
            if not isinstance(d, torch.Tensor):
                cache = self.__dict__.setdefault("_der_consts", {})
                key = (float(d), str(self.device))
                if key not in cache:
                    cache[key] = vl.from_numpy(np.array([[float(d)]], np.float32), self.device)
                d = cache[key]
            self.vars[k].der = d
        if not self.accumulateParamDers and self._flat is None:
            for p in self.params.values():
                p.der = None
        self._pending_param_ders = {}
        hooks = self.bwdHooks
        for step in reversed(plan):
            if hooks:
                h = hooks.get(step.rec.name)
                if h is not None:
                    h()
            step.backward(self)
        mark("bwd1")
        if self._side_pending:
            torch.cuda.current_stream().wait_stream(self.wgradStream)
            self._side_pending = False
        mark("join")

    def _set_var_der(self, name, d):
        if d is None:
            return
        v = self.vars[name]
        if v.der is None:
            v.der = d
        else:
            v.der = vl.sum2(v.der, d)

    def _direct_der(self, rec):
        if self._flat is None or self.accumulateParamDers:
            return None
        ps = [self.params[p] for p in rec.params]
        if any(p.fanout > 1 or p.der is None for p in ps):
            return None
        return [p.der for p in ps]

    def _set_param_der(self, name, d):
        if d is None:
            return
        p = self.params[name]
        if self._flat is not None and d is p.der:
            return
        seen = self._pending_param_ders.get(name, 0)
        self._pending_param_ders[name] = seen + 1
        if self._flat is not None:
            if seen == 0 and not self.accumulateParamDers:
                p.der.copy_(d)
            else:
                p.der.add_(d)
        else:
            p.der = d if (p.der is None or seen == 0 and not self.accumulateParamDers) else vl.sum2(p.der, d)

    def _plan(self, training):
        key = (training, self.mode, self.fuse, len(self.layers),
               tuple(n for n, v in self.vars.items() if v.precious))
        if getattr(self, "_plan_key", None) == key and getattr(self, "_plan_layers", None) == [
                id(l) for l in self.layers]:
            return self._plan_cache
        steps = build_plan(self, training)
        self._plan_key, self._plan_cache = key, steps
        self._plan_layers = [id(l) for l in self.layers]
        return steps


class FlatParams:
    def __init__(self, val, der, mom, segments):
        self.val, self.der, self.mom, self.segments = val, der, mom, segments


class _Step:

    def __init__(self, rec):
        self.rec = rec
        self.bias_from = None
        self.moments_for = None
        self.bias_conv = None
        self.bias_conv_done = False
        self.se_bn = None
        self.stem_into = None

    def _bias_der_slot(self, net):
        self.bias_conv_done = False
        if self.bias_conv is None or net._flat is None or net.accumulateParamDers or not net.fuseBiasDer:
            return None
        if net.wgradStream is not None and type(self) is not _BnReluPoolStep:
            return None
        bp = net.params[self.bias_conv.rec.params[1]]
        if bp.fanout == 1 and bp.der is not None:
            self.bias_conv_done = True
            return bp.der
        return None

    def _params(self, net):
        return [net.params[p].value for p in self.rec.params]

    def forward(self, net):
        r = self.rec
        if self.se_bn is not None and self.se_bn.fwd is not None and isinstance(r.block, GlobalPooling):
            f = self.se_bn.fwd
            net.vars[r.outputs[0]].value = vl.se_squeeze_bn(f["u"], f["g"], f["b"], f["moments"])
            return
        if self.stem_into is not None and self.stem_into.stem_forward(net, self):
            return
        ins = [net.vars[v].value for v in r.inputs]
        if net._training and net.wgradStream is not None and isinstance(r.block, Conv) and \
                net.vars[r.inputs[0]].fanin > 0 and net.prepareBackward:
            with torch.cuda.stream(net.wgradStream):
                vl.conv_prepare_backward(ins[0], self._params(net)[0], stride=r.block.stride, pad=r.block.pad,
                                         dilate=r.block.dilate)
        bn = self.moments_for
        if bn is not None and net._training and net.mode != "test" and net.fuseStats:
            do = net._direct_der(bn)
            mo = do[2] if do else vl.mat_empty(bn.block.numChannels, 2, device=ins[0].device)
            prm = self._params(net)
            blk = r.block
            outs = [vl.vl_nnconv(ins[0], prm[0], prm[1] if blk.hasBias else None, stride=blk.stride, pad=blk.pad,
                                 dilate=blk.dilate, moments_out=mo, epsilon=bn.block.epsilon)]
            bn.block._pre_moments = mo
        else:
            outs = r.block.forward(ins, self._params(net))
        for v, t in zip(r.outputs, outs):
            net.vars[v].value = t

    def backward(self, net):
        r = self.rec
        douts = [net.vars[v].der for v in r.outputs]
        if all(d is None for d in douts):
            return
        ins = [net.vars[v].value for v in r.inputs]
        if isinstance(r.block, Conv):
            need_dx = net.vars[r.inputs[0]].fanin > 0
            skip_db = self.bias_from is not None and self.bias_from.bias_conv_done
            side = net.wgradStream if need_dx else None
            if side is not None and net._flat is not None and net._direct_der(r) is None:
                side = None
            xin = net.vars[r.inputs[0]]
            accum = xin.der if need_dx else None
            if accum is not None:
                xin.der = None
            if side is None:
                dins, dpar = r.block.backward(ins, self._params(net), douts, need_dx=need_dx,
                                              der_out=net._direct_der(r), skip_db=skip_db, dx_accum=accum)
                if net.gradHook is not None:
                    if net._side_pending:
                        torch.cuda.current_stream().wait_stream(net.wgradStream)
                    net.gradHook(r.name)
            else:
                main = torch.cuda.current_stream()
                defer = net.wgradAfterDgrad
                if defer:
                    dins, _ = r.block.backward(ins, self._params(net), douts, need_dx=True, need_df=False,
                                               dx_accum=accum)
                side.wait_stream(main)
                with torch.cuda.stream(side):
                    _, dpar = r.block.backward(ins, self._params(net), douts, need_dx=False,
                                               der_out=net._direct_der(r), skip_db=skip_db)
                    if net.gradHook is not None:
                        net.gradHook(r.name)
                douts[0].record_stream(side)
                ins[0].record_stream(side)
                net._side_pending = True
                if not defer:
                    dins, _ = r.block.backward(ins, self._params(net), douts, need_dx=True, need_df=False,
                                               dx_accum=accum)
            if skip_db:
                dpar = [dpar[0], net.params[r.params[1]].der]
        elif isinstance(r.block, BatchNorm):
            dins, dpar = r.block.backward(ins, self._params(net), douts, der_out=net._direct_der(r),
                                          dxsum_out=self._bias_der_slot(net))
        elif isinstance(r.block, GlobalPooling) and self.se_bn is not None and self.se_bn.stash is not None:
            self.se_bn.stash["dgp"] = douts[0]
            if net.conserveMemory:
                for v in r.outputs:
                    if not net.vars[v].precious:
                        net.vars[v].der = None
            return
        elif isinstance(r.block, GlobalPooling) and r.block.method == "avg" and net.vars[r.inputs[0]].der is not None \
                and net.fuseForkSums:
            xin = net.vars[r.inputs[0]]
            acc, xin.der = xin.der, None
            dins, dpar = [vl.vl_nnpool(ins[0], [int(ins[0].shape[0]), int(ins[0].shape[1])], douts[0], method="avg",
                                       dx_accum=acc)], []
        elif isinstance(r.block, Pooling):
            outs = [net.vars[v].value for v in r.outputs]
            dins, dpar = r.block.backward(ins, self._params(net), douts,
                                          outputs=outs if outs[0] is not None else None)
        else:
            dins, dpar = r.block.backward(ins, self._params(net), douts)
        for v, d in zip(r.inputs, dins):
            net._set_var_der(v, d)
        for p, d in zip(r.params, dpar):
            net._set_param_der(p, d)
# ... 256 lines not shown
        side = net.wgradStream
        main = torch.cuda.current_stream()
        if side is not None:
            side.wait_stream(main)
        with torch.cuda.stream(side if side is not None else main):
            res = None
            if net.fuseStemGram or fwd is not None:
                cpar = cs._params(net)
                res = vl.conv_backward_filter_bnrelupool_gram(
                    xin, cpar[0], cpar[1] if blk.hasBias else None, g, moments, am, None if fwd is not None else out.value,
                    out.der, pb.poolSize, stride=blk.stride, pad=blk.pad, dilate=blk.dilate, pool_stride=pb.stride,
                    pool_pad=pb.pad, train=not test, gram=fwd["gram"] if fwd is not None else None, df_out=cdo[0],
                    dbias_out=cdo[1] if blk.hasBias else None, dg_out=do[0], db_out=do[1])
                if res is None and fwd is not None:
                    raise RuntimeError("fused stem: the library took the forward call but not the backward one (%s)" % cr.name)
            if res is None:
                res = vl.conv_backward_filter_bnrelupool(
                    xin, blk.size, x, g, b, moments, am, out.value, out.der, pb.poolSize, stride=blk.stride, pad=blk.pad,
                    dilate=blk.dilate, pool_stride=pb.stride, pool_pad=pb.pad, train=not test, df_out=cdo[0],
                    dbias_out=cdo[1] if blk.hasBias else None, dg_out=do[0], db_out=do[1], has_bias=blk.hasBias)
            if res is not None and net.gradHook is not None:
                if side is None and net._side_pending:
                    main.wait_stream(net.wgradStream)
                net.gradHook(cr.name)
        if res is None:
            self._stem_fused = False
            return False
        if side is not None:
            for t in (xin, x, am, out.value, out.der, moments) + ((fwd["gram"],) if fwd is not None else ()):
                if t is not None:
                    t.record_stream(side)
            net._side_pending = True
        self.bias_conv_done = True
        return True


class _ConvActStep(_Step):

    def __init__(self, conv_rec, act_rec):
        super().__init__(conv_rec)
        self.act_rec = act_rec

    def forward(self, net):
        r, blk = self.rec, self.rec.block
        par = self._params(net)
        sig = isinstance(self.act_rec.block, Sigmoid)
        y = vl.vl_nnconv(net.vars[r.inputs[0]].value, par[0], par[1] if blk.hasBias else None, stride=blk.stride,
                         pad=blk.pad, dilate=blk.dilate, relu=not sig, sigmoid=sig)
        net.vars[self.act_rec.outputs[0]].value = y

    def backward(self, net):
        raise RuntimeError("dagnn: a forward-only plan was asked for derivatives")


class _ConvFoldStep(_Step):

    def __init__(self, conv_rec, bn_rec, sum_rec, relu_rec, out_name):
        super().__init__(conv_rec)
        self.bn_rec, self.sum_rec, self.relu_rec, self.out_name = bn_rec, sum_rec, relu_rec, out_name
        self._folded = None

    def _fold(self, net):
        g, b, mom = [net.params[p].value for p in self.bn_rec.params]
        key = (g.data_ptr(), b.data_ptr(), mom.data_ptr(), g._version, b._version, mom._version,
               net.paramGeneration)
        if self._folded is None or self._folded[0] != key:
            gn, bn_, mn = vl.to_numpy(g).ravel(), vl.to_numpy(b).ravel(), vl.to_numpy(mom)
            sc = (gn / mn[:, 1]).astype(np.float32)
            sh = (bn_ - mn[:, 0] * sc).astype(np.float32)
            self._folded = (key, vl.from_numpy(sc.reshape(-1, 1), g.device),
                            vl.from_numpy(sh.reshape(-1, 1), g.device))
        return self._folded[1], self._folded[2]

    def forward(self, net):
        r = self.rec
        blk = r.block
        x = net.vars[r.inputs[0]].value
        prm = self._params(net)
        sc, sh = self._fold(net)
        resid = None
        if self.sum_rec is not None:
            other = [v for v in self.sum_rec.inputs if v != self.bn_rec.outputs[0]][0]
            resid = net.vars[other].value
        y = vl.vl_nnconv(x, prm[0], prm[1] if blk.hasBias else None, stride=blk.stride, pad=blk.pad,
                         dilate=blk.dilate, scale=sc, shift=sh, residual=resid,
                         relu=self.relu_rec is not None)
        net.vars[self.out_name].value = y

    def backward(self, net):
        raise RuntimeError("folded conv+bn steps exist only in forward-only test-mode plans")


class _SEFoldStep(_ConvFoldStep):

    def __init__(self, conv_rec, bn_rec, se):
        super().__init__(conv_rec, bn_rec, None, se["relu"], se["out"])
        self.se = se
        self._reduce = None

    def _fold_reduce(self, net, F, bias, sc, sh, F1, b1):
        ts = [t for t in (F, bias, sc, sh, F1, b1) if t is not None]
        key = tuple(t.data_ptr() for t in ts) + tuple(t._version for t in ts) + (net.paramGeneration,)
        if self._reduce is None or self._reduce[0] != key:
            Kp, Cc = int(F.shape[2]), int(F.shape[3])
            Fm = vl.to_numpy(F).astype(np.float64).reshape(Kp, Cc, order="F")
            F1m = vl.to_numpy(F1).astype(np.float64).reshape(Cc, int(F1.shape[3]), order="F")
            scn, shn = vl.to_numpy(sc).astype(np.float64).ravel(), vl.to_numpy(sh).astype(np.float64).ravel()
            bn_ = vl.to_numpy(bias).astype(np.float64).ravel() if bias is not None else np.zeros(Cc)
            f10 = (Fm * scn[None, :]) @ F1m
            b10 = F1m.T @ (scn * bn_ + shn)
            if b1 is not None:
                b10 = b10 + vl.to_numpy(b1).astype(np.float64).ravel()
            self._reduce = (key,
                            vl.from_numpy(np.asfortranarray(f10.astype(np.float32).reshape(1, 1, Kp, -1, order="F")), F.device),
                            vl.from_numpy(b10.astype(np.float32).reshape(-1, 1), F.device))
        return self._reduce[1], self._reduce[2]

    def forward(self, net):
        r, blk, se = self.rec, self.rec.block, self.se
        u = net.vars[r.inputs[0]].value
        prm = self._params(net)
        bias = prm[1] if blk.hasBias else None
        sc, sh = self._fold(net)
        ubar = vl.vl_nnpool(u, [int(u.shape[0]), int(u.shape[1])], method="avg")
        f1 = [net.params[p].value for p in se["fc1"].params]
        f2 = [net.params[p].value for p in se["fc2"].params]
        b1 = f1[1] if se["fc1"].block.hasBias else None
        if net.foldSEReduce:
            f10, b10 = self._fold_reduce(net, prm[0], bias, sc, sh, f1[0], b1)
            h = vl.vl_nnconv(ubar, f10, b10, relu=True)
        else:
            z = vl.vl_nnconv(ubar, prm[0], bias, scale=sc, shift=sh)
            h = vl.vl_nnconv(z, f1[0], b1, relu=True)
        a = vl.vl_nnconv(h, f2[0], f2[1] if se["fc2"].block.hasBias else None, sigmoid=True)
        y = vl.vl_nnconv(u, prm[0], bias, stride=blk.stride, pad=blk.pad, dilate=blk.dilate, scale=sc, shift=sh,
                         gate=a, residual=net.vars[se["shortcut"]].value, relu=se["relu"] is not None)
        net.vars[self.out_name].value = y


def _match_se_tail(net, recs, consumers, order, conv_rec, bn_rec, keep_values=False):
    blk = conv_rec.block
    if blk.size[0] != 1 or blk.size[1] != 1 or tuple(vl._pair(blk.stride, "STRIDE")) != (1, 1) or any(vl._pad4(blk.pad)):
        return None
    x = bn_rec.outputs[0]
    cs = consumers.get(x, [])
    if len(cs) != 2 or net.vars[x].precious:
        return None
    gp = [c for c in cs if isinstance(c.block, GlobalPooling) and c.block.method == "avg"]
    ax = [c for c in cs if isinstance(c.block, Axpy)]
    if len(gp) != 1 or len(ax) != 1:
        return None
    gp, ax = gp[0], ax[0]

    def only(var, cls):
        c = consumers.get(var, [])
        return c[0] if len(c) == 1 and isinstance(c[0].block, cls) and (keep_values or not net.vars[var].precious) else None
    fc1 = only(gp.outputs[0], Conv)
    r1 = only(fc1.outputs[0], ReLU) if fc1 else None
    fc2 = only(r1.outputs[0], Conv) if r1 else None
    sg = only(fc2.outputs[0], Sigmoid) if fc2 else None
    if sg is None or r1.block.leak != 0.0 or only(sg.outputs[0], Axpy) is not ax:
        return None
    for fc in (fc1, fc2):
        b = fc.block
        if b.size[0] != 1 or b.size[1] != 1 or tuple(vl._pair(b.stride, "STRIDE")) != (1, 1) or any(vl._pad4(b.pad)):
            return None
# ... 144 lines not shown
```

### mcncrossmodalemotions_amd/train.py

```python
import ctypes as C
import pickle

import numpy as np
import torch

from . import _lib, vl


class TrainOpts:
    def __init__(self, learningRate=None, momentum=0.9, weightDecay=5e-4, batchSize=64,
                 derOutputs=("objective", 1)):
        self.learningRate = np.logspace(-4, -5, 300) if learningRate is None else np.atleast_1d(learningRate)
        self.momentum = momentum
        self.weightDecay = weightDecay
        self.batchSize = batchSize
        self.derOutputs = list(derOutputs)


class ParameterServer:

    def __init__(self, backend="torch"):
        self.backend = backend
        self.world = 1
        self.rank = 0
# ... 195 lines not shown
        for l in net.layers:
            if isinstance(l.block, dagnn.Conv):
                p = net.params[l.params[0]]
                if p.fanout == 1 and hasattr(p, "_flat_off"):
                    n = (int(p.value.numel()) + 3) // 4 * 4
                    items.append((p._flat_off, p._flat_off + n, l.name))
        items.sort()
        runs, cur = [], []
        for it in items:
            if cur and it[0] != cur[-1][1]:
                runs.append(cur)
                cur = []
            cur.append(it)
        if cur:
            runs.append(cur)
        self.buckets = []
        for run in runs:
            acc = []
            for it in reversed(run):
                acc.append(it)
                if 4 * (acc[0][1] - acc[-1][0]) >= target_bytes:
                    self.buckets.append((acc[-1][0], acc[0][1], min((x[2] for x in acc), key=lambda n: order[n])))
                    acc = []
            if acc:
                self.buckets.append((acc[-1][0], acc[0][1], min((x[2] for x in acc), key=lambda n: order[n])))
        self.buckets.sort(key=lambda x: -order[x[2]])
        self.by_trigger = {}
        for a, b, t in self.buckets:
            self.by_trigger.setdefault(t, []).append((a, b))
        covered = sorted((a, b) for a, b, _ in self.buckets)
        self.rest, pos = [], 0
        for a, b in covered:
            if a > pos:
                self.rest.append((pos, a))
            pos = b
        if pos < total:
            self.rest.append((pos, total))
        self._sent = set()
        self.log = None

    def ranges(self):
        return [(a, b) for a, b, _ in self.buckets] + self.rest

    def begin(self):
        self._sent = set()

    def _push(self, parserv, a, b):
        if self.log is not None:
            self.log.append((a, b))
        parserv.push(self.flat.der[a:b])

    def on_layer(self, parserv, name):
        for a, b in self.by_trigger.get(name, ()):
            self._sent.add((a, b))
            self._push(parserv, a, b)

    def finish(self, parserv):
        for a, b, _ in self.buckets:
            if (a, b) not in self._sent:
                self._push(parserv, a, b)
        for a, b in self.rest:
            self._push(parserv, a, b)
        parserv.sync()


def _in_buckets(buckets, a, b):
    return any(x < b and a < y for x, y, _ in buckets.buckets)


def shard_batch(batch, rank, world):
    return list(batch)[rank::world]


def accumulate_gradients(net, opts, lr, global_batch, moments_denom=1.0):
    flat = net._flat
    for (method, lr_mult, wd_mult), a, b in flat.segments:
        if b == a:
            continue
        if method == "average":
            vl.average_update(flat.val[a:b], flat.der[a:b], lr_mult, moments_denom)
        else:
            vl.sgd_update(flat.val[a:b], flat.mom[a:b], flat.der[a:b], lr * lr_mult, opts.momentum,
                          opts.weightDecay * wd_mult, global_batch)
    net.paramGeneration = getattr(net, "paramGeneration", 0) + 1


def train_step(net, inputs, opts, epoch=0, parserv=None, global_batch=None, input_events=None, local_batch=None):
    if net._flat is None:
        net.pack_params()
    net.mode = "normal"
    world = parserv.world if parserv is not None else 1
    exchange = parserv is not None and parserv.active
    global_batch = global_batch or opts.batchSize
    if local_batch is None:
        local_batch = 0 if inputs is None else global_batch / world
    buckets = None
    if exchange and parserv.overlap:
        buckets = net.__dict__.get("_grad_buckets")
        if buckets is None or buckets.flat is not net._flat:
            buckets = net.__dict__["_grad_buckets"] = GradBuckets(net)
        buckets.begin()
    net.gradHook = None
    if buckets is not None and inputs is not None and not any(m == "average" for (m, _, _), a, b in net._flat.segments
                                                              if b > a and _in_buckets(buckets, a, b)):
        net.gradHook = lambda name: buckets.on_layer(parserv, name)
    if inputs is None:
        net._flat.der.zero_()
    else:
        net.eval(inputs, opts.derOutputs, input_events=input_events)
    if exchange:
        for (method, _, _), a, b in net._flat.segments:
            if method == "average" and b > a:
                vl.scale_(net._flat.der[a:b], float(local_batch))
        if buckets is not None:
            buckets.finish(parserv)
        else:
            parserv.allreduce_(net._flat.der)
    net.gradHook = None
    lr = float(opts.learningRate[min(epoch, len(opts.learningRate) - 1)])
    accumulate_gradients(net, opts, lr, global_batch, float(global_batch) if exchange else 1.0)
    if net.markHook is not None:
        net.markHook("upd")


def extractStats(stats, net):
    from . import dagnn
    stats = dict(stats or {})
    for l in net.layers:
        b = l.block
        if not isinstance(b, dagnn.LossBase):
            continue
        if isinstance(b, dagnn.ErrorStats):
            metrics, dist = b.average, b.classDist
            pop = dist / dist.sum() if dist.sum() > 0 else dist
            names = (net.meta.get("classes", {}).get("name") or
                     ["class%d" % (i + 1) for i in range(len(metrics))])
            stats["meanAcc"] = float(np.mean(metrics))
            for name, m in zip(names, metrics):
                stats[name] = float(m)
            for name, q in zip(names, pop):
                stats["%sPop" % name] = float(q)
        else:
            if b.ignoreAverage:
                continue
            stats[l.outputs[0]] = b.average
    return stats


def _reset_losses(net):
    from . import dagnn
    for l in net.layers:
        if isinstance(l.block, dagnn.LossBase):
            l.block.reset()


class _RunAhead:

    def __init__(self, device):
        self.on = device is not None and device.type == "cuda"
        self.inflight = []

    def tick(self):
        if not self.on:
            return
        ev = torch.cuda.Event()
        ev.record()
        self.inflight.append(ev)
# ... 179 lines not shown
```

### mcncrossmodalemotions_amd/vl.py

```python
import ctypes as C

import numpy as np
import torch

from . import _lib



def _dev():
    return torch.device("cuda", torch.cuda.current_device())


XM_ENOTSUP = 5


def mat_empty(*shape, device=None):
    shape = tuple(int(s) for s in (shape[0] if len(shape) == 1 and not np.isscalar(shape[0]) else shape))
    t = torch.empty(tuple(reversed(shape)), dtype=torch.float32, device=device or _dev())
    return t.permute(*reversed(range(len(shape))))


def mat_zeros(*shape, device=None):
    t = mat_empty(*shape, device=device)
    t.zero_()
# ... 82 lines not shown


def set_exec_hint(flags):
    old = int(_L().xm_get_exec_hint())
    _lib.check(_L().xm_set_exec_hint(int(flags)))
    return old


def out_size(n, pa, pb, f, d, s):
    return _L().xm_out_size(n, pa, pb, f, d, s)




def vl_nnconv(x, f, b=None, dzdy=None, stride=1, pad=0, dilate=1, no_der_data=False,
              no_der_filters=False, no_der_biases=False, scale=None, shift=None, residual=None,
              relu=False, df_out=None, db_out=None, dx_accum=None, sigmoid=False, moments_out=None, epsilon=1e-4,
              gate=None):
    x, f = _chk(x, "X"), _chk(f, "F")
    H, W, Cc, N = _shape4(x)
    FH, FW, FC, K = _shape4(f)
    sy, sx = _pair(stride, "STRIDE")
    dy, dx = _pair(dilate, "DILATE")
    pt, pb, pl, pr = _pad4(pad)
    bb = None
    if b is not None and b.numel() > 0:
        bb = _chk(b, "B")
        if bb.numel() != K:
            raise ValueError("vl_nnconv: B has %d elements, expected %d" % (bb.numel(), K))
    L = _L()
    Ho = L.xm_out_size(H, pt, pb, FH, dy, sy)
    Wo = L.xm_out_size(W, pl, pr, FW, dx, sx)
    if dzdy is None:
        y = mat_empty(max(Ho, 0), max(Wo, 0), K, N, device=x.device)
        fused = scale is not None or residual is not None or relu or sigmoid
        if gate is not None:
            gt = _chk(gate, "GATE")
            if gt.numel() != K * N:
                raise ValueError("vl_nnconv: GATE must be 1 x 1 x %d x %d" % (K, N))
            if residual is not None and _shape4(_chk(residual, "RESIDUAL")) != [Ho, Wo, K, N]:
                raise ValueError("vl_nnconv: residual shape mismatch")
            _lib.check(L.xm_nnconv_forward_gated(
                _ptr(x), H, W, Cc, N, _ptr(f), FH, FW, FC, K, _ptr(bb), _ptr(y), sy, sx, pt, pb, pl, pr, dy, dx,
                _ptr(scale), _ptr(shift), _ptr(gt), _ptr(residual), (1 if relu else 0) | (4 if sigmoid else 0), _stream()))
        elif moments_out is not None:
            if fused:
                raise ValueError("vl_nnconv: moments_out cannot be combined with a fused epilogue")
            mo = _chk(moments_out, "MOMENTS")
            if mo.numel() != 2 * K:
                raise ValueError("vl_nnconv: moments_out must be %d x 2" % K)
            _lib.check(L.xm_nnconv_forward_moments(_ptr(x), H, W, Cc, N, _ptr(f), FH, FW, FC, K, _ptr(bb), _ptr(y),
                                                   sy, sx, pt, pb, pl, pr, dy, dx, float(epsilon), _ptr(mo),
                                                   _stream()))
        elif fused:
            if residual is not None:
                _chk(residual, "RESIDUAL")
                if _shape4(residual) != [Ho, Wo, K, N]:
                    raise ValueError("vl_nnconv: residual shape mismatch")
            _lib.check(L.xm_nnconv_forward_fused(
                _ptr(x), H, W, Cc, N, _ptr(f), FH, FW, FC, K, _ptr(bb), _ptr(y), sy, sx, pt, pb,
                pl, pr, dy, dx, _ptr(scale), _ptr(shift), _ptr(residual), (1 if relu else 0) | (4 if sigmoid else 0),
                _stream()))
        else:
            _lib.check(L.xm_nnconv_forward(_ptr(x), H, W, Cc, N, _ptr(f), FH, FW, FC, K, _ptr(bb),
                                           _ptr(y), sy, sx, pt, pb, pl, pr, dy, dx, _stream()))
        return y
    dzdy = _chk(dzdy, "DZDY")
    if _shape4(dzdy) != [Ho, Wo, K, N]:
        raise ValueError("vl_nnconv: DZDY is %r, expected %r" % (tuple(dzdy.shape), (Ho, Wo, K, N)))
    dxo = None if no_der_data else mat_empty(H, W, Cc, N, device=x.device)
    dfo = None if no_der_filters else (df_out if df_out is not None else mat_empty(FH, FW, FC, K, device=x.device))
    dbo = None if (no_der_biases or bb is None) else (db_out if db_out is not None else mat_empty(K, 1, device=x.device))
    acc = None
    if dx_accum is not None and dxo is not None:
        acc = _chk(dx_accum, "DX_ACCUM")
        if _shape4(acc) != [H, W, Cc, N]:
            raise ValueError("vl_nnconv: dx_accum must have the size of X")
    _lib.check(L.xm_nnconv_backward_accum(_ptr(x), H, W, Cc, N, _ptr(f), FH, FW, FC, K, _ptr(dzdy),
                                          _ptr(dxo), _ptr(dfo), _ptr(dbo), sy, sx, pt, pb, pl, pr, dy, dx,
                                          _ptr(acc), _stream()))
    return dxo, dfo, dbo


def conv_prepare_backward(x, f, stride=1, pad=0, dilate=1):
    H, W, Cc, N = _shape4(x)
    FH, FW, FC, K = _shape4(f)
    sy, sx = _pair(stride, "STRIDE")
    dy, dx = _pair(dilate, "DILATE")
    pt, pb, pl, pr = _pad4(pad)
    _lib.check(_L().xm_nnconv_prepare_backward(H, W, Cc, N, _ptr(f), FH, FW, FC, K, sy, sx, pt, pb, pl, pr, dy, dx,
                                               _stream()))


_METHOD = {"max": 0, "avg": 1}


def vl_nnpool(x, pool, dzdy=None, stride=1, pad=0, method="max", argmax=None, want_argmax=False, dx_accum=None):
    x = _chk(x, "X")
    if method not in _METHOD:
        raise ValueError("vl_nnpool: unknown METHOD '%s'" % method)
    H, W, Cc, N = _shape4(x)
    ph, pw = _pair(pool, "POOL")
    sy, sx = _pair(stride, "STRIDE")
    pt, pb, pl, pr = _pad4(pad)
    L = _L()
    Ho = L.xm_out_size(H, pt, pb, ph, 1, sy)
    Wo = L.xm_out_size(W, pl, pr, pw, 1, sx)
    if dzdy is None:
        y = mat_empty(max(Ho, 0), max(Wo, 0), Cc, N, device=x.device)
        if want_argmax and method == "max":
            am = torch.empty(max(Ho, 0) * max(Wo, 0) * Cc * N, dtype=torch.uint8, device=x.device)
            _lib.check(L.xm_nnpool_forward_argmax(_ptr(x), H, W, Cc, N, ph, pw, sy, sx, pt, pb, pl, pr,
                                                  _ptr(y), C.c_void_p(am.data_ptr()), _stream()))
            return y, am
        _lib.check(L.xm_nnpool_forward(_ptr(x), H, W, Cc, N, ph, pw, sy, sx, pt, pb, pl, pr,
                                       _METHOD[method], _ptr(y), _stream()))
        return (y, None) if want_argmax else y
    dzdy = _chk(dzdy, "DZDY")
    if _shape4(dzdy) != [Ho, Wo, Cc, N]:
        raise ValueError("vl_nnpool: DZDY is %r, expected %r" % (tuple(dzdy.shape), (Ho, Wo, Cc, N)))
    dxo = mat_empty(H, W, Cc, N, device=x.device)
    if dx_accum is not None:
        if method != "avg" or (ph, pw) != (H, W) or (pt | pb | pl | pr) or _shape4(dx_accum) != [H, W, Cc, N]:
            raise ValueError("vl_nnpool: dx_accum is built for global average pooling only")
        _lib.check(L.xm_nnpool_global_avg_backward_accum(_ptr(dzdy), _ptr(_chk(dx_accum, "DX_ACCUM")), _ptr(dxo), H, W, Cc, N,
                                                         _stream()))
        return dxo
    if argmax is not None and method == "max":
        _lib.check(L.xm_nnpool_backward_argmax(C.c_void_p(argmax.data_ptr()), H, W, Cc, N, ph, pw, sy,
                                               sx, pt, pb, pl, pr, _ptr(dzdy), _ptr(dxo), _stream()))
    else:
        _lib.check(L.xm_nnpool_backward(_ptr(x), H, W, Cc, N, ph, pw, sy, sx, pt, pb, pl, pr,
                                        _METHOD[method], _ptr(dzdy), _ptr(dxo), _stream()))
    return dxo




def vl_nnbnorm(x, g, b, dzdy=None, epsilon=1e-4, moments=None, relu=False, y=None, dg_out=None,
               db_out=None, moments_out=None, batch_moments=False, dxsum_out=None):
    x, g, b = _chk(x, "X"), _chk(g, "G"), _chk(b, "B")
    H, W, Cc, N = _shape4(x)
    if g.numel() != Cc or b.numel() != Cc:
        raise ValueError("vl_nnbnorm: G and B must have %d elements" % Cc)
    mi = None
    if moments is not None:
        mi = _chk(moments, "MOMENTS")
        if mi.numel() != 2 * Cc:
            raise ValueError("vl_nnbnorm: MOMENTS must be %d x 2" % Cc)
    L = _L()
    mo = moments_out if moments_out is not None else mat_empty(Cc, 2, device=x.device)
    if dzdy is None:
        yo = mat_empty(H, W, Cc, N, device=x.device)
        _lib.check(L.xm_nnbnorm_forward_fused(_ptr(x), H, W, Cc, N, _ptr(g), _ptr(b),
                                              float(epsilon), _ptr(mi), _ptr(yo), _ptr(mo),
                                              1 if relu else 0, _stream()))
        return yo, mo
    dzdy = _chk(dzdy, "DZDY")
    if _shape4(dzdy) != [H, W, Cc, N]:
        raise ValueError("vl_nnbnorm: DZDY shape mismatch")
    dxo = mat_empty(H, W, Cc, N, device=x.device)
    dg = dg_out if dg_out is not None else mat_empty(Cc, 1, device=x.device)
    db = db_out if db_out is not None else mat_empty(Cc, 1, device=x.device)
    if batch_moments and mi is None:
        raise ValueError("vl_nnbnorm: batch_moments needs the moments of the forward call")
    if dxsum_out is not None:
        if relu and y is None:
            raise ValueError("vl_nnbnorm: fused backward needs the forward output y")
        if _chk(dxsum_out, "DXSUM").numel() != Cc:
            raise ValueError("vl_nnbnorm: dxsum_out must have %d elements" % Cc)
        _lib.check(L.xm_nnbnorm_backward_dxsum(_ptr(x), _ptr(_chk(y, "Y")) if relu else None, H, W, Cc, N,
                                               _ptr(g), _ptr(b), _ptr(dzdy), float(epsilon), _ptr(mi),
                                               _ptr(dxo), _ptr(dg), _ptr(db), _ptr(mo), _ptr(dxsum_out),
                                               (1 if relu else 0) | (2 if batch_moments else 0), _stream()))
# ... 1045 lines not shown
```

Measured before the change: 4086 pairs/s.

## Cache padded and dgrad filter relayouts, refresh all in one batched kernel after SGD

Filter relayouts (forward padding and dgrad transpose/prep) are now cached per weight buffer and tracked with a 'current' flag instead of a global version counter. After each SGD or average update, one relayout_batch_kernel regenerates every cached relayout overlapping the updated weights, replacing many small per-layer launches. Forward convs reuse the cached padded filter, and the dgrad prepare on the side stream is skipped when already current. This adds bookkeeping, a binary-search dispatch inside the kernel, and stream-event dependencies, and carries a staleness risk if weights change outside the hooked paths.

```diff
diff --git a/include/xmodal.h b/include/xmodal.h
--- a/include/xmodal.h
+++ b/include/xmodal.h
@@ -61,6 +61,9 @@
                        int dx, void *stream);
 int xm_nnconv_prepare_backward(int H, int W, int C, int N, const float *f, int FH, int FW, int FC, int K,
                                int sy, int sx, int pt, int pb, int pl, int pr, int dy, int dx, void *stream);
+int xm_nnconv_backward_prepared(int H, int W, int C, int N, const float *f, int FH, int FW, int FC, int K,
+                                int sy, int sx, int pt, int pb, int pl, int pr, int dy, int dx);
+int xm_nnconv_prepare_forward(const float *f, int FH, int FW, int FC, int K, void *stream);
 int xm_params_changed(void);
 int xm_nnconv_backward_accum(const float *x, int H, int W, int C, int N, const float *f, int FH, int FW,
                              int FC, int K, const float *dzdy, float *dx_out, float *df_out,
diff --git a/mcncrossmodalemotions_amd/_lib.py b/mcncrossmodalemotions_amd/_lib.py
--- a/mcncrossmodalemotions_amd/_lib.py
+++ b/mcncrossmodalemotions_amd/_lib.py
@@ -46,6 +46,8 @@
                                                  [c_fp, c_fp] + [_i] * 9 + [c_fp, c_fp, c_fp, _vp, c_fp, c_fp, c_fp, c_fp, _vp],
     "xm_nnconv_bnorm_relu_pool_forward": [c_fp] + [_i] * 4 + [c_fp] + [_i] * 4 + [c_fp] + [_i] * 8 + [c_fp, c_fp, _f, c_fp] +
                                          [_i] * 8 + [_vp, c_fp, c_fp, c_fp, _vp],
+    "xm_nnconv_backward_prepared": [_i] * 4 + [c_fp] + [_i] * 12,
+    "xm_nnconv_prepare_forward": [c_fp] + [_i] * 4 + [_vp],
     "xm_params_changed": [],
     "xm_nnpool_forward": [c_fp] + [_i] * 13 + [c_fp, _vp],
     "xm_nnpool_backward": [c_fp] + [_i] * 13 + [c_fp, c_fp, _vp],
diff --git a/mcncrossmodalemotions_amd/csrc/context.cpp b/mcncrossmodalemotions_amd/csrc/context.cpp
--- a/mcncrossmodalemotions_amd/csrc/context.cpp
+++ b/mcncrossmodalemotions_amd/csrc/context.cpp
@@ -94,7 +94,7 @@
 
 extern "C" {
 
-int xm_version(void) { return 114; }
+int xm_version(void) { return 115; }
 const char *xm_last_error(void) { return xm::err_buf(); }
 
 int xm_workspace_reserve(size_t bytes) {
diff --git a/mcncrossmodalemotions_amd/csrc/conv.hip b/mcncrossmodalemotions_amd/csrc/conv.hip
--- a/mcncrossmodalemotions_amd/csrc/conv.hip
+++ b/mcncrossmodalemotions_amd/csrc/conv.hip
@@ -13,25 +13,28 @@
 namespace xm {
 
 
-__global__ void pad_filter_kernel(const float *__restrict__ f, float *__restrict__ o, int M, int R,
-                                  int Rp) {
-  size_t i = blockIdx.x * (size_t)blockDim.x + threadIdx.x;
+__device__ __forceinline__ void pad_filter_body(const float *__restrict__ f, float *__restrict__ o, int M, int R, int Rp,
+                                                unsigned block) {
+  size_t i = block * (size_t)256 + threadIdx.x;
   if (i >= (size_t)M * Rp) return;
   int r = (int)(i % Rp);
   size_t m = i / Rp;
   o[i] = r < R ? f[m * R + r] : 0.f;
 }
+__global__ void __launch_bounds__(256)
+pad_filter_kernel(const float *__restrict__ f, float *__restrict__ o, int M, int R, int Rp) {
+  pad_filter_body(f, o, M, R, Rp, blockIdx.x);
+}
 
 struct PrepDiv {
   FastDiv tsT, T, tsNT, nT, nU, padc, rows;
 };
-__global__ void __launch_bounds__(256)
-prep_dgrad_filter_kernel(const float *__restrict__ f, float *__restrict__ o, int FH, int FW, int FC,
-                         int Kg, int u0, int ustep, int nU, int v0, int vstep, int nV, int lda,
-                         int TS, int fold, PrepDiv dv) {
-  extern __shared__ float tile[];
+__device__ __forceinline__ void
+prep_dgrad_filter_body(const float *__restrict__ f, float *__restrict__ o, int FH, int FW, int FC,
+                       int Kg, int u0, int ustep, int nU, int v0, int vstep, int nV, int lda,
+                       int TS, int fold, const PrepDiv dv, int bx, int by, float *tile) {
   const int T = FH * FW, nT = nU * nV;
-  const int c0 = blockIdx.x * TS, k0 = blockIdx.y * TS;
+  const int c0 = bx * TS, k0 = by * TS;
   const int pitch = TS * T + 1;
   for (int i = threadIdx.x; i < TS * TS * T; i += 256) {
     int kl = (int)xm_div((uint32_t)i, dv.tsT), rem = i - kl * (TS * T);
@@ -52,7 +55,7 @@
       o[dst] = tile[kl * pitch + cl * T + t];
     }
   }
-  if (blockIdx.y == 0) {
+  if (by == 0) {
     const int used = (fold ? nV : nT) * Kg, rows = fold ? nU : 1;
     int padc = lda - used;
     for (int i = threadIdx.x; i < TS * rows * padc; i += 256) {
@@ -62,11 +65,17 @@
     }
   }
 }
-
 __global__ void __launch_bounds__(256)
-transpose_filter_kernel(const float *__restrict__ f, float *__restrict__ o, int K, int R, int ldo) {
-  __shared__ float tile[64][65];
-  const int r0 = blockIdx.x * 64, k0 = blockIdx.y * 64;
+prep_dgrad_filter_kernel(const float *__restrict__ f, float *__restrict__ o, int FH, int FW, int FC,
+                         int Kg, int u0, int ustep, int nU, int v0, int vstep, int nV, int lda,
+                         int TS, int fold, PrepDiv dv) {
+  extern __shared__ float tile[];
+  prep_dgrad_filter_body(f, o, FH, FW, FC, Kg, u0, ustep, nU, v0, vstep, nV, lda, TS, fold, dv, blockIdx.x, blockIdx.y, tile);
+}
+
+__device__ __forceinline__ void transpose_filter_body(const float *__restrict__ f, float *__restrict__ o, int K, int R,
+                                                      int ldo, int bx, int by, float (*tile)[65]) {
+  const int r0 = bx * 64, k0 = by * 64;
   const int tx = threadIdx.x & 15, ty = threadIdx.x >> 4;
 #pragma unroll
   for (int p = 0; p < 4; ++p) {
@@ -88,6 +97,40 @@
       *reinterpret_cast<float4 *>(o + (size_t)r * ldo + k) = v;
     }
   }
+}
+__global__ void __launch_bounds__(256)
+transpose_filter_kernel(const float *__restrict__ f, float *__restrict__ o, int K, int R, int ldo) {
+  __shared__ float tile[64][65];
+  transpose_filter_body(f, o, K, R, ldo, blockIdx.x, blockIdx.y, tile);
+}
+
+enum { kRelayPrep = 0, kRelayTranspose = 1, kRelayPad = 2 };
+struct RelayoutRow {
+  const float *src;
+  float *dst;
+  int kind, block0, gx;
+  int a[13];
+  PrepDiv dv;
+};
+__global__ void __launch_bounds__(256)
+relayout_batch_kernel(const RelayoutRow *__restrict__ rows, int nrows) {
+  extern __shared__ float lds[];
+  const int b = (int)blockIdx.x;
+  int lo = 0, hi = nrows - 1;
+  while (lo < hi) {
+    const int mid = (lo + hi + 1) >> 1;
+    if (rows[mid].block0 <= b) lo = mid; else hi = mid - 1;
+  }
+  const RelayoutRow &r = rows[lo];
+  const int lb = b - r.block0, by = lb / r.gx, bx = lb - by * r.gx;
+  const int *a = r.a;
+  if (r.kind == kRelayPrep)
+    prep_dgrad_filter_body(r.src, r.dst, a[0], a[1], a[2], a[3], a[4], a[5], a[6], a[7], a[8], a[9], a[10], a[11], a[12],
+                           r.dv, bx, by, lds);
+  else if (r.kind == kRelayTranspose)
+    transpose_filter_body(r.src, r.dst, a[0], a[1], a[2], bx, by, reinterpret_cast<float (*)[65]>(lds));
+  else
+    pad_filter_body(r.src, r.dst, a[0], a[1], a[2], (unsigned)lb);
 }
 
 template <int ZL>
@@ -1211,6 +1254,172 @@
   return arm(select_arm(4, key, st, 4, hok, kHaloMargin, halo_forced(hok), arm));
 }
 
+struct PrepKey {
+  const float *f;
+  int FH, FW, FC, K, sy, sx, dy, dx, pt, pl, H, W, fold;
+  bool operator<(const PrepKey &o) const { return memcmp(this, &o, sizeof(PrepKey)) < 0; }
+};
+struct RowPlan {
+  RelayoutRow r;
+  int gy;
+  size_t lds;
+};
+struct PrepEntry {
+  float *buf = nullptr;
+  size_t bytes = 0;
+  bool current = false;
+  hipEvent_t ev = nullptr;
+  hipEvent_t ready = nullptr;
+  hipStream_t st = nullptr;
+  const char *src = nullptr;
+  size_t src_bytes = 0;
+  std::vector<RowPlan> rows;
+};
+static std::map<PrepKey, PrepEntry> g_prep;
+static unsigned long long g_prep_gen = 1;
+static int g_relayout_launches = 0, g_relayout_batches = 0;
+static const size_t kRelayoutMaxLds = 64 * 1024;
+static PrepKey prep_key(const float *f, const Geo &g, bool fold) {
+  PrepKey k;
+  memset(&k, 0, sizeof k);
+  k.f = f, k.FH = g.FH, k.FW = g.FW, k.FC = g.FC, k.K = g.K, k.sy = g.sy, k.sx = g.sx, k.dy = g.dy, k.dx = g.dx;
+  k.pt = g.pt, k.pl = g.pl, k.H = g.H, k.W = g.W, k.fold = fold ? 1 : 0;
+  return k;
+}
+static PrepKey pad_key(const float *f, int FH, int FW, int FC, int K) {
+  PrepKey k;
+  memset(&k, 0, sizeof k);
+  k.f = f, k.FH = FH, k.FW = FW, k.FC = FC, k.K = K, k.fold = 2;
+  return k;
+}
+static PrepEntry *prep_find_current(const PrepKey &key) {
+  auto it = g_prep.find(key);
+  return (it != g_prep.end() && it->second.current) ? &it->second : nullptr;
+}
+static int prep_register(const PrepKey &key, size_t bytes, const float *f, size_t filter_floats, PrepEntry **out) {
+  PrepEntry *pe = &g_prep[key];
+  if (pe->bytes < bytes) {
+    if (pe->buf) {
+      XM_HIP(hipDeviceSynchronize());
+      (void)hipFree(pe->buf);
+    }
+    pe->buf = nullptr;
+    pe->current = false;
+    XM_HIP(hipMalloc((void **)&pe->buf, bytes));
+    pe->bytes = bytes;
+    ++g_prep_gen;
+  }
+  if (!pe->ev) XM_HIP(hipEventCreateWithFlags(&pe->ev, hipEventDisableTiming));
+  pe->src = (const char *)f, pe->src_bytes = filter_floats * sizeof(float);
+  *out = pe;
+  return XM_OK;
+}
+static int launch_row(const RowPlan &p, hipStream_t st) {
+  const RelayoutRow &r = p.r;
+  const int *a = r.a;
+  ++g_relayout_launches;
+  if (r.kind == kRelayTranspose)
+    hipLaunchKernelGGL(transpose_filter_kernel, dim3(r.gx, p.gy), dim3(256), 0, st, r.src, r.dst, a[0], a[1], a[2]);
+  else if (r.kind == kRelayPrep)
+    hipLaunchKernelGGL(prep_dgrad_filter_kernel, dim3(r.gx, p.gy), dim3(256), p.lds, st, r.src, r.dst, a[0], a[1], a[2],
+                       a[3], a[4], a[5], a[6], a[7], a[8], a[9], a[10], a[11], a[12], r.dv);
+  else
+    hipLaunchKernelGGL(pad_filter_kernel, dim3(r.gx), dim3(256), 0, st, r.src, r.dst, a[0], a[1], a[2]);
+  XM_LAUNCH_CHECK();
+  return XM_OK;
+}
+static RowPlan pad_filter_row(const float *f, float *Ap, int M, int R, int Rp) {
+  RowPlan p{};
+  p.r.src = f, p.r.dst = Ap, p.r.kind = kRelayPad;
+  p.r.gx = (int)(((size_t)M * Rp + 255) / 256), p.gy = 1;
+  p.r.a[0] = M, p.r.a[1] = R, p.r.a[2] = Rp;
+  return p;
+}
+static int prep_stamp(PrepEntry *pe, hipStream_t st) {
+  pe->current = true;
+  pe->st = st;
+  pe->ready = pe->ev;
+  XM_HIP(hipEventRecord(pe->ev, st));
+  return XM_OK;
+}
+static int prep_consume(const PrepEntry *pe, hipStream_t st) {
+  if (pe->st != st) XM_HIP(hipStreamWaitEvent(st, pe->ready, 0));
+  return XM_OK;
+}
+
+struct RelayoutBatch {
+  unsigned long long gen = 0;
+  std::vector<PrepEntry *> members, stale;
+  RelayoutRow *dev = nullptr, *host = nullptr;
+  size_t cap = 0, lds = 0;
+  int nrows = 0, nblocks = 0;
+  hipEvent_t ev = nullptr, copied = nullptr;
+  hipStream_t st = nullptr;
+  bool launched = false;
+};
+static std::map<std::pair<const void *, size_t>, RelayoutBatch> g_batches;
+static int relayout_batch_rebuild(RelayoutBatch &B, const char *w, size_t bytes, hipStream_t st) {
+  B.members.clear(), B.stale.clear();
+  std::vector<RelayoutRow> rows;
+  B.nblocks = 0, B.lds = 0;
+  for (auto &kv : g_prep) {
+    PrepEntry *pe = &kv.second;
+    if (!pe->buf || pe->src + pe->src_bytes <= w || w + bytes <= pe->src) continue;
+    if (pe->rows.empty()) {
+      B.stale.push_back(pe);
+      continue;
+    }
+    B.members.push_back(pe);
+    for (const RowPlan &p : pe->rows) {
+      RelayoutRow r = p.r;
+      r.block0 = B.nblocks;
+      B.nblocks += r.gx * p.gy;
+      B.lds = std::max(B.lds, p.lds);
+      rows.push_back(r);
+    }
+  }
+  B.nrows = (int)rows.size();
+  if (!B.ev) {
+    XM_HIP(hipEventCreateWithFlags(&B.ev, hipEventDisableTiming));
+    XM_HIP(hipEventCreateWithFlags(&B.copied, hipEventDisableTiming));
+  }
+  if (rows.size() > B.cap) {
+    size_t cap = 64;
+    while (cap < rows.size()) cap *= 2;
+    XM_HIP(hipMalloc((void **)&B.dev, cap * sizeof(RelayoutRow)));
+    XM_HIP(hipHostMalloc((void **)&B.host, cap * sizeof(RelayoutRow), hipHostMallocDefault));
+    B.cap = cap;
+  } else if (B.launched) {
+    XM_HIP(hipEventSynchronize(B.copied));
+    if (B.st != st) XM_HIP(hipStreamWaitEvent(st, B.ev, 0));
+  }
+  if (!rows.empty()) {
+    memcpy(B.host, rows.data(), rows.size() * sizeof(RelayoutRow));
+    XM_HIP(hipMemcpyAsync(B.dev, B.host, rows.size() * sizeof(RelayoutRow), hipMemcpyHostToDevice, st));
+    XM_HIP(hipEventRecord(B.copied, st));
+  }
+  B.gen = g_prep_gen;
+  return XM_OK;
+}
+int params_updated(const void *w, size_t bytes, hipStream_t st) {
+  if (g_prep.empty() || !w || !bytes) return XM_OK;
+  RelayoutBatch &B = g_batches[std::make_pair(w, bytes)];
+  if (B.gen != g_prep_gen) {
+    int rc = relayout_batch_rebuild(B, (const char *)w, bytes, st);
+    if (rc) return rc;
+  }
+  for (PrepEntry *pe : B.stale) pe->current = false;
+  if (B.members.empty()) return XM_OK;
+  if (B.launched && B.st != st) XM_HIP(hipStreamWaitEvent(st, B.ev, 0));
+  hipLaunchKernelGGL(relayout_batch_kernel, dim3((unsigned)B.nblocks), dim3(256), B.lds, st, B.dev, B.nrows);
+  XM_LAUNCH_CHECK();
+  ++g_relayout_batches;
+  XM_HIP(hipEventRecord(B.ev, st));
+  B.st = st, B.launched = true;
+  for (PrepEntry *pe : B.members) pe->current = true, pe->st = st, pe->ready = B.ev;
+  return XM_OK;
+}
+
 static int conv_forward(const float *x, const float *f, const float *b, float *y, const Geo &g,
                         const float *scale, const float *shift, const float *resid, int relu,
                         hipStream_t st, float *moments_out = nullptr, float eps = 0.f, const float *gate = nullptr) {
@@ -1230,18 +1439,22 @@
   const bool want_stats = moments_out != nullptr && g.G == 1 && path_on(kPathFusedStats);
   const size_t statf = want_stats ? (size_t)2 * g.K * std::max((NP + 31) / 32, stem_grid(NP)) : 0;
   const size_t stat2 = want_stats ? (size_t)2 * g.K * 64 : 0;
+  PrepEntry *padded_f = need_pad ? prep_find_current(pad_key(f, g.FH, g.FW, g.FC, g.K)) : nullptr;
   WsCarver ws;
-  int rc = ws.init(WsCarver::need(need_pad ? (size_t)g.K * Rp : 0, 4) + WsCarver::need(slabf, 4) +
+  int rc = ws.init(WsCarver::need(need_pad && !padded_f ? (size_t)g.K * Rp : 0, 4) + WsCarver::need(slabf, 4) +
                        WsCarver::need(statf, 4) + WsCarver::need(stat2, 8), st);
   if (rc) return rc;
   FwdOperands o{x, f, b, scale, shift, resid, gate, y, device_taps(fwd_tap_table(g, Rp, bigTaps)), g.R, Rp, relu, bigTaps, dma_ok};
   if (!o.taps) return fail(XM_ENOMEM, "vl_nnconv: tap table allocation failed");
-  if (need_pad) {
+  if (padded_f) {
+    rc = prep_consume(padded_f, st);
+    if (rc) return rc;
+    o.A = padded_f->buf;
+    o.lda = Rp;
+  } else if (need_pad) {
     float *Ap = ws.take<float>((size_t)g.K * Rp);
-    size_t n = (size_t)g.K * Rp;
-    hipLaunchKernelGGL(pad_filter_kernel, dim3((unsigned)((n + 255) / 256)), dim3(256), 0, st, f, Ap,
-                       g.K, g.R, Rp);
-    XM_LAUNCH_CHECK();
+    rc = launch_row(pad_filter_row(f, Ap, g.K, g.R, Rp), st);
+    if (rc) return rc;
     o.A = Ap;
     o.lda = Rp;
   }
@@ -1263,28 +1476,6 @@
   }
   if (moments_out && !stats_done) return bn_batch_moments(y, g.Ho, g.Wo, g.K, g.N, eps, moments_out, st);
   return XM_OK;
-}
-
-struct PrepKey {
-  const float *f;
-  int FH, FW, FC, K, sy, sx, dy, dx, pt, pl, H, W, fold;
-  bool operator<(const PrepKey &o) const { return memcmp(this, &o, sizeof(PrepKey)) < 0; }
-};
-struct PrepEntry {
-  float *buf = nullptr;
-  size_t bytes = 0;
-  unsigned long long version = ~0ull;
-  hipEvent_t ev = nullptr;
-  hipStream_t st = nullptr;
-};
-static std::map<PrepKey, PrepEntry> g_prep;
-unsigned long long g_param_version = 1;
-static PrepKey prep_key(const float *f, const Geo &g, bool fold) {
-  PrepKey k;
-  memset(&k, 0, sizeof k);
-  k.f = f, k.FH = g.FH, k.FW = g.FW, k.FC = g.FC, k.K = g.K, k.sy = g.sy, k.sx = g.sx, k.dy = g.dy, k.dx = g.dx;
-  k.pt = g.pt, k.pl = g.pl, k.H = g.H, k.W = g.W, k.fold = fold ? 1 : 0;
-  return k;
 }
 
 static int g_force_dgrad_s2 = -1;
@@ -1346,29 +1537,30 @@
          (Rrows & 3) == 0 && (g.Kg & 3) == 0 && g.G == 1 && (((uintptr_t)f | (uintptr_t)Ag) & 15) == 0 &&
          path_on(kPathFastTranspose);
 }
-static int launch_dgrad_filter(const float *f, float *Ag, const Geo &g, const DgradClass &c, int grp, bool foldH, hipStream_t st) {
+static RowPlan dgrad_filter_row(const float *f, float *Ag, const Geo &g, const DgradClass &c, int grp, bool foldH) {
+  RowPlan p{};
+  p.r.dst = Ag;
   if (dgrad_pure_transpose(g, c, foldH, f, Ag)) {
     const int Rrows = g.FC * (foldH ? g.FH : 1);
-    hipLaunchKernelGGL(transpose_filter_kernel, dim3((Rrows + 63) / 64, (g.Kg + 63) / 64), dim3(256), 0, st, f, Ag,
-                       g.Kg, Rrows, c.Rp);
-    XM_LAUNCH_CHECK();
-    return XM_OK;
+    p.r.src = f, p.r.kind = kRelayTranspose;
+    p.r.gx = (Rrows + 63) / 64, p.gy = (g.Kg + 63) / 64, p.lds = sizeof(float) * 64 * 65;
+    p.r.a[0] = g.Kg, p.r.a[1] = Rrows, p.r.a[2] = c.Rp;
+    return p;
   }
   const int T = g.FH * g.FW;
   const int TS = T <= 14 ? 32 : (T <= 56 ? 16 : 8);
-  size_t lds = sizeof(float) * (size_t)TS * (TS * T + 1);
   const int nT = c.nU * c.nV, used = (foldH ? c.nV : nT) * g.Kg;
-  PrepDiv pd;
+  PrepDiv &pd = p.r.dv;
   pd.tsT = make_fastdiv((uint32_t)(TS * T)), pd.T = make_fastdiv((uint32_t)T);
   pd.tsNT = make_fastdiv((uint32_t)std::max(1, TS * nT)), pd.nT = make_fastdiv((uint32_t)std::max(1, nT));
   pd.nU = make_fastdiv((uint32_t)std::max(1, c.nU));
   pd.padc = make_fastdiv((uint32_t)std::max(1, c.Rp - used));
   pd.rows = make_fastdiv((uint32_t)(foldH ? std::max(1, c.nU) : 1));
-  hipLaunchKernelGGL(prep_dgrad_filter_kernel, dim3((g.FC + TS - 1) / TS, (g.Kg + TS - 1) / TS),
-                     dim3(256), lds, st, f + (size_t)g.R * g.Kg * grp, Ag, g.FH, g.FW, g.FC, g.Kg,
-                     c.u0, c.ustep, c.nU, c.v0, c.vstep, c.nV, c.Rp, TS, foldH ? 1 : 0, pd);
-  XM_LAUNCH_CHECK();
-  return XM_OK;
+  p.r.src = f + (size_t)g.R * g.Kg * grp, p.r.kind = kRelayPrep;
+  p.r.gx = (g.FC + TS - 1) / TS, p.gy = (g.Kg + TS - 1) / TS, p.lds = sizeof(float) * (size_t)TS * (TS * T + 1);
+  const int args[13] = {g.FH, g.FW, g.FC, g.Kg, c.u0, c.ustep, c.nU, c.v0, c.vstep, c.nV, c.Rp, TS, foldH ? 1 : 0};
+  memcpy(p.r.a, args, sizeof args);
+  return p;
 }
 
 static int dgrad_filter_operand(const float *f, const Geo &g, const std::vector<DgradClass> &cls, bool foldH,
@@ -1381,39 +1573,37 @@
   const PrepKey pkey = prep_key(f, g, foldH);
   PrepEntry *pe = nullptr;
   bool have_prepared = false;
+  int rc;
   if (prepare_only) {
-    pe = &g_prep[pkey];
-    if (pe->bytes < abytes) {
-      if (pe->buf) {
-        XM_HIP(hipDeviceSynchronize());
-        (void)hipFree(pe->buf);
-      }
-      pe->buf = nullptr;
-      XM_HIP(hipMalloc((void **)&pe->buf, abytes));
-      pe->bytes = abytes;
-    }
-    if (!pe->ev) XM_HIP(hipEventCreateWithFlags(&pe->ev, hipEventDisableTiming));
+    rc = prep_register(pkey, abytes, f, (size_t)g.R * g.K, &pe);
+    if (rc) return rc;
   } else {
-    auto it = g_prep.find(pkey);
-    if (it != g_prep.end() && it->second.version == g_param_version && it->second.bytes >= abytes) {
-      pe = &it->second;
+    pe = prep_find_current(pkey);
+    if (pe && pe->bytes < abytes) pe = nullptr;
+    if (pe) {
       have_prepared = true;
-      if (pe->st != st) XM_HIP(hipStreamWaitEvent(st, pe->ev, 0));
-    }
-  }
-  int rc = ws.init((pe ? 0 : abytes) + WsCarver::need(slab_floats, 4), st);
+      rc = prep_consume(pe, st);
+      if (rc) return rc;
+    }
+  }
+  rc = ws.init((pe ? 0 : abytes) + WsCarver::need(slab_floats, 4), st);
   if (rc) return rc;
   F.base = pe ? (char *)pe->buf : ws.base;
   F.slab = slab_floats ? (float *)(ws.base + (pe ? 0 : abytes)) : nullptr;
+  std::vector<RowPlan> rows;
+  bool batchable = true;
   for (size_t ic = 0; ic < cls.size() && !have_prepared; ++ic)
     for (int grp = 0; grp < g.G; ++grp) {
-      rc = launch_dgrad_filter(f, F.of(g, cls[ic], ic, grp, foldH), g, cls[ic], grp, foldH, st);
+      rows.push_back(dgrad_filter_row(f, F.of(g, cls[ic], ic, grp, foldH), g, cls[ic], grp, foldH));
+      batchable = batchable && rows.back().lds <= kRelayoutMaxLds;
+      rc = launch_row(rows.back(), st);
       if (rc) return rc;
     }
   if (prepare_only) {
-    pe->version = g_param_version;
-    pe->st = st;
-    XM_HIP(hipEventRecord(pe->ev, st));
+    if (!batchable) rows.clear();
+    if (pe->rows.size() != rows.size()) ++g_prep_gen;
+    pe->rows = rows;
+    return prep_stamp(pe, st);
   }
   return XM_OK;
 }
@@ -1519,6 +1709,7 @@
     return launch_dgrad_s2(dzdy, f, dxo, g, st);
   }
   const bool foldH = dgrad_fold_h(g);
+  if (prepare_only && prep_find_current(prep_key(f, g, foldH))) return XM_OK;
   bool covers_all = true;
   const std::vector<DgradClass> cls = dgrad_classes(g, foldH, &covers_all);
   if (!prepare_only && (!covers_all || cls.empty())) {
@@ -1865,6 +2056,8 @@
 }
 int xm_debug_get(const char *key) {
   if (key && strcmp(key, "num_conv_cfgs") == 0) return kNumCfg;
+  if (key && strcmp(key, "relayout_launches") == 0) return g_relayout_launches;
+  if (key && strcmp(key, "relayout_batches") == 0) return g_relayout_batches;
   const DebugSwitch *s = debug_switch(key);
   return s ? *s->value : INT_MIN;
 }
@@ -2104,8 +2297,32 @@
   return conv_dgrad(f, nullptr, nullptr, g, (hipStream_t)stream, nullptr, true);
 }
 
+int xm_nnconv_backward_prepared(int H, int W, int C, int N, const float *f, int FH, int FW, int FC, int K,
+                                int sy, int sx, int pt, int pb, int pl, int pr, int dy, int dx) {
+  Geo g;
+  if (!f || make_geo(g, H, W, C, N, FH, FW, FC, K, sy, sx, pt, pb, pl, pr, dy, dx)) return 0;
+  if (dgrad_s2_ok(g, nullptr, nullptr, nullptr)) return 1;
+  return prep_find_current(prep_key(f, g, dgrad_fold_h(g))) ? 1 : 0;
+}
+
+int xm_nnconv_prepare_forward(const float *f, int FH, int FW, int FC, int K, void *stream) {
+  if (!f) return fail(XM_EINVAL, "vl_nnconv: F is NULL");
+  if (FH <= 0 || FW <= 0 || FC <= 0 || K <= 0 || too_big(FH, FW, FC, K)) return fail(XM_EINVAL, "vl_nnconv: bad filter size");
+  const int R = FH * FW * FC, Rp = (R + kBK - 1) / kBK * kBK;
+  if (R % kBK == 0 && ((uintptr_t)f & 15) == 0) return XM_OK;
+  const PrepKey key = pad_key(f, FH, FW, FC, K);
+  if (prep_find_current(key)) return XM_OK;
+  PrepEntry *pe = nullptr;
+  int rc = prep_register(key, WsCarver::need((size_t)K * Rp, 4), f, (size_t)R * K, &pe);
+  if (rc) return rc;
+  if (pe->rows.empty()) ++g_prep_gen;
+  pe->rows.assign(1, pad_filter_row(f, pe->buf, K, R, Rp));
+  rc = launch_row(pe->rows[0], (hipStream_t)stream);
+  return rc ? rc : prep_stamp(pe, (hipStream_t)stream);
+}
+
 int xm_params_changed(void) {
-  ++g_param_version;
+  for (auto &kv : g_prep) kv.second.current = false;
   return XM_OK;
 }
 
diff --git a/mcncrossmodalemotions_amd/csrc/misc.hip b/mcncrossmodalemotions_amd/csrc/misc.hip
--- a/mcncrossmodalemotions_amd/csrc/misc.hip
+++ b/mcncrossmodalemotions_amd/csrc/misc.hip
@@ -1,7 +1,7 @@
 #include "xm_common.h"
 
 namespace xm {
-extern unsigned long long g_param_version;
+int params_updated(const void *w, size_t bytes, hipStream_t st);
 }
 
 namespace xm {
@@ -789,7 +789,6 @@
 
 int xm_sgd_update(float *w, float *m, const float *der, size_t n, float lr, float momentum,
                   float weight_decay, float batch, void *stream) {
-  ++xm::g_param_version;
   if (n == 0) return XM_OK;
   if (!w || !m || !der) return fail(XM_EINVAL, "sgd: NULL tensor");
   if (!(batch > 0.f)) return fail(XM_EINVAL, "sgd: batch must be > 0");
@@ -797,7 +796,7 @@
   hipLaunchKernelGGL(sgd_kernel, dim3(ew_grid(vec ? n / 4 + 1 : n)), dim3(256), 0, (hipStream_t)stream,
                      w, m, der, n, lr, momentum, weight_decay, 1.0f / batch, vec);
   XM_LAUNCH_CHECK();
-  return XM_OK;
+  return xm::params_updated(w, n * sizeof(float), (hipStream_t)stream);
 }
 
 int xm_scale_f32(float *x, size_t n, float a, void *stream) {
@@ -829,13 +828,12 @@
 }
 
 int xm_average_update(float *w, const float *der, size_t n, float lr, float nworkers, void *stream) {
-  ++xm::g_param_version;
   if (n == 0) return XM_OK;
   if (!w || !der) return fail(XM_EINVAL, "average update: NULL tensor");
   hipLaunchKernelGGL(average_kernel, dim3((unsigned)((n + 255) / 256)), dim3(256), 0,
                      (hipStream_t)stream, w, der, n, lr, 1.0f / nworkers);
   XM_LAUNCH_CHECK();
-  return XM_OK;
+  return xm::params_updated(w, n * sizeof(float), (hipStream_t)stream);
 }
 
 __global__ void __launch_bounds__(256)
diff --git a/mcncrossmodalemotions_amd/dagnn.py b/mcncrossmodalemotions_amd/dagnn.py
--- a/mcncrossmodalemotions_amd/dagnn.py
+++ b/mcncrossmodalemotions_amd/dagnn.py
@@ -443,6 +443,11 @@
     @paramGeneration.setter
     def paramGeneration(self, v):
         self._gen[0] = int(v)
+        if self.device is not None and self.device.type == "cuda":
+            vl.params_changed()
+
+    def _params_updated(self):
+        self._gen[0] += 1
 
     def addLayer(self, name, block, inputs, outputs, params=()):
         if isinstance(inputs, str):
@@ -571,6 +576,7 @@
         for p in self.params.values():
             if p.value is not None and not isinstance(p.value, torch.Tensor):
                 p.value = vl.from_numpy(p.value, self.device)
+        self.paramGeneration += 1
         return self
 
     def pack_params(self):
@@ -616,8 +622,7 @@
             self.vars[k].value = t
         plan = self._plan(derOutputs is not None)
         self._training = derOutputs is not None
-        if self._training and self.wgradStream is not None:
-            self.wgradStream.wait_stream(torch.cuda.current_stream())
+        self._side_joined = False
         pending = dict(input_events or {})
         mark = self.markHook or (lambda label: None)
         mark("fwd0")
@@ -659,6 +664,18 @@
             self._side_pending = False
         mark("join")
 
+    def _prepare_dgrad(self, x, f, blk):
+        if vl.conv_backward_prepared(x, f, stride=blk.stride, pad=blk.pad, dilate=blk.dilate):
+            return
+        if self.wgradStream is None:
+            vl.conv_prepare_backward(x, f, stride=blk.stride, pad=blk.pad, dilate=blk.dilate)
+            return
+        if not self._side_joined:
+            self.wgradStream.wait_stream(torch.cuda.current_stream())
+            self._side_joined = True
+        with torch.cuda.stream(self.wgradStream):
+            vl.conv_prepare_backward(x, f, stride=blk.stride, pad=blk.pad, dilate=blk.dilate)
+
     def _set_var_der(self, name, d):
         if d is None:
             return
@@ -702,6 +719,11 @@
         self._plan_key, self._plan_cache = key, steps
         self._plan_layers = [id(l) for l in self.layers]
         return steps
+
+
+def _reads_padded_filter(blk):
+    sz = blk.size
+    return (int(sz[0]) * int(sz[1]) * int(sz[2])) % 16 != 0
 
 
 class FlatParams:
@@ -744,11 +766,11 @@
         if self.stem_into is not None and self.stem_into.stem_forward(net, self):
             return
         ins = [net.vars[v].value for v in r.inputs]
-        if net._training and net.wgradStream is not None and isinstance(r.block, Conv) and \
-                net.vars[r.inputs[0]].fanin > 0 and net.prepareBackward:
-            with torch.cuda.stream(net.wgradStream):
-                vl.conv_prepare_backward(ins[0], self._params(net)[0], stride=r.block.stride, pad=r.block.pad,
-                                         dilate=r.block.dilate)
+        if net._training and isinstance(r.block, Conv) and net.vars[r.inputs[0]].fanin > 0 and net.prepareBackward \
+                and ins[0].is_cuda:
+            net._prepare_dgrad(ins[0], self._params(net)[0], r.block)
+        if isinstance(r.block, Conv) and _reads_padded_filter(r.block) and ins[0].is_cuda:
+            vl.conv_prepare_forward(self._params(net)[0])
         bn = self.moments_for
         if bn is not None and net._training and net.mode != "test" and net.fuseStats:
             do = net._direct_der(bn)
@@ -1171,6 +1193,8 @@
         if self.sum_rec is not None:
             other = [v for v in self.sum_rec.inputs if v != self.bn_rec.outputs[0]][0]
             resid = net.vars[other].value
+        if _reads_padded_filter(blk) and x.is_cuda:
+            vl.conv_prepare_forward(prm[0])
         y = vl.vl_nnconv(x, prm[0], prm[1] if blk.hasBias else None, stride=blk.stride, pad=blk.pad,
                          dilate=blk.dilate, scale=sc, shift=sh, residual=resid,
                          relu=self.relu_rec is not None)
diff --git a/mcncrossmodalemotions_amd/train.py b/mcncrossmodalemotions_amd/train.py
--- a/mcncrossmodalemotions_amd/train.py
+++ b/mcncrossmodalemotions_amd/train.py
@@ -301,7 +301,7 @@
         else:
             vl.sgd_update(flat.val[a:b], flat.mom[a:b], flat.der[a:b], lr * lr_mult, opts.momentum,
                           opts.weightDecay * wd_mult, global_batch)
-    net.paramGeneration = getattr(net, "paramGeneration", 0) + 1
+    net._params_updated()
 
 
 def train_step(net, inputs, opts, epoch=0, parserv=None, global_batch=None, input_events=None, local_batch=None):
diff --git a/mcncrossmodalemotions_amd/vl.py b/mcncrossmodalemotions_amd/vl.py
--- a/mcncrossmodalemotions_amd/vl.py
+++ b/mcncrossmodalemotions_amd/vl.py
@@ -188,14 +188,30 @@
     return dxo, dfo, dbo
 
 
-def conv_prepare_backward(x, f, stride=1, pad=0, dilate=1):
+def _prepare_args(x, f, stride, pad, dilate):
     H, W, Cc, N = _shape4(x)
     FH, FW, FC, K = _shape4(f)
     sy, sx = _pair(stride, "STRIDE")
     dy, dx = _pair(dilate, "DILATE")
     pt, pb, pl, pr = _pad4(pad)
-    _lib.check(_L().xm_nnconv_prepare_backward(H, W, Cc, N, _ptr(f), FH, FW, FC, K, sy, sx, pt, pb, pl, pr, dy, dx,
-                                               _stream()))
+    return (H, W, Cc, N, _ptr(f), FH, FW, FC, K, sy, sx, pt, pb, pl, pr, dy, dx)
+
+
+def conv_prepare_backward(x, f, stride=1, pad=0, dilate=1):
+    _lib.check(_L().xm_nnconv_prepare_backward(*_prepare_args(x, f, stride, pad, dilate), _stream()))
+
+
+def conv_backward_prepared(x, f, stride=1, pad=0, dilate=1):
+    return bool(_L().xm_nnconv_backward_prepared(*_prepare_args(x, f, stride, pad, dilate)))
+
+
+def conv_prepare_forward(f):
+    FH, FW, FC, K = _shape4(f)
+    _lib.check(_L().xm_nnconv_prepare_forward(_ptr(f), FH, FW, FC, K, _stream()))
+
+
+def params_changed():
+    _lib.check(_L().xm_params_changed())
 
 
 _METHOD = {"max": 0, "avg": 1}
```

Result: no change. 4080 pairs/s (-0.1%).
